# SayanoAI/Comfy-RVC

Hardware: AMD Instinct MI355X
Metric: audio-sec/wall-sec (xRT), 40k_v2 end-to-end VC (higher is better)
Workload: dtype f32; 1 GPU; Full VC 40k_v2 (HuBERT -> RMVPE -> SynthesizerTrnMs768NSFsid), 30 s 16 kHz clips, 12 per GPU per step (3 in flight), vc_single host array in -> int16 host array out (BASELINE.json configs[2]); clips_in_flight_per_gpu=3, weights=procedural (comfy-rvc_amd/synthetic.py), noise=device generator, seeded per clip, parallelism=clip-per-GPU x1 (3 lanes each), one RCCL gather of the step's int16 waveforms

## Files before the change

### comfy-rvc_amd/_lib.py

```python
import ctypes as C
import os

_HERE = os.path.dirname(os.path.abspath(__file__))
LIB_PATH = os.environ.get("RVC_HIP_LIB") or os.path.join(_HERE, "csrc", "librvc_hip.so")


class RvcHipError(RuntimeError):
    pass


def _load():
    if not os.path.isfile(LIB_PATH):
        raise RvcHipError(
            f"{LIB_PATH} is missing: build it with `python -c 'import __graft_entry__ as g; g.build()'` "
            "(or `make -C comfy-rvc_amd/csrc`).  There is no CPU fallback.")
    return C.CDLL(LIB_PATH)


lib = _load()

c_void_p, c_int, c_int64, c_float, c_char_p = C.c_void_p, C.c_int, C.c_int64, C.c_float, C.c_char_p
P = C.POINTER


# ... 38 lines not shown


SIGNATURES = {
    "rvc_last_error": (c_char_p, []),
    "rvc_version": (c_char_p, []),
    "rvc_ctx_create": (c_int, [c_int, P(c_void_p)]),
    "rvc_ctx_destroy": (c_int, [c_void_p]),
    "rvc_ctx_workspace_bytes": (c_int64, [c_void_p]),
    "rvc_ctx_set_conv_precision": (c_int, [c_void_p, c_int]),
    "rvc_hubert_create": (c_int, [c_void_p, P(c_void_p)]),
    "rvc_hubert_set_tensor": (c_int, [c_void_p, c_char_p, c_void_p, P(c_int64), c_int]),
    "rvc_hubert_finalize": (c_int, [c_void_p]),
    "rvc_hubert_destroy": (c_int, [c_void_p]),
    "rvc_hubert_num_frames": (c_int64, [c_int64]),
    "rvc_hubert_forward": (c_int, [c_void_p, c_void_p, c_void_p, c_int64, c_int, c_int, c_void_p, c_void_p, P(HubertTaps)]),
    "rvc_rmvpe_create": (c_int, [c_void_p, P(c_void_p)]),
    "rvc_rmvpe_set_tensor": (c_int, [c_void_p, c_char_p, c_void_p, P(c_int64), c_int]),
    "rvc_rmvpe_finalize": (c_int, [c_void_p]),
    "rvc_rmvpe_destroy": (c_int, [c_void_p]),
    "rvc_rmvpe_forward": (c_int, [c_void_p, c_void_p, c_void_p, c_int64, c_float, c_void_p, c_void_p, c_void_p, P(RmvpeTaps)]),
    "rvc_f0_post": (c_int, [c_void_p, c_void_p, c_int64, C.c_double, C.c_double, C.c_double, c_int, c_void_p, c_void_p]),
    "rvc_rmvpe_decode": (c_int, [c_void_p, c_void_p, c_void_p, c_int64, c_float, c_void_p]),
    "rvc_rmvpe_status": (c_int, [c_void_p, c_void_p]),
    "rvc_rmvpe_debug_fault": (c_int, [c_void_p, c_int, C.c_uint]),
    "rvc_rmvpe_repaired": (c_int, [c_void_p, c_void_p]),
    "rvc_crepe_create": (c_int, [c_void_p, c_int, P(c_void_p)]),
    "rvc_crepe_set_tensor": (c_int, [c_void_p, c_char_p, c_void_p, P(c_int64), c_int]),
    "rvc_crepe_finalize": (c_int, [c_void_p]),
    "rvc_crepe_destroy": (c_int, [c_void_p]),
    "rvc_crepe_num_frames": (c_int64, [c_int64, c_int, c_int]),
    "rvc_crepe_forward": (c_int, [c_void_p, c_void_p, c_void_p, c_int64, c_int, c_int, c_void_p, P(CrepeTaps)]),
    "rvc_crepe_viterbi": (c_int, [c_void_p, c_void_p, c_int64, c_int, c_int, c_void_p, c_void_p]),
    "rvc_mdx23_create": (c_int, [c_void_p, P(Mdx23Config), P(c_void_p)]),
    "rvc_mdx23_set_tensor": (c_int, [c_void_p, c_char_p, c_void_p, P(c_int64), c_int]),
    "rvc_mdx23_finalize": (c_int, [c_void_p]),
    "rvc_mdx23_destroy": (c_int, [c_void_p]),
    "rvc_mdx23_forward": (c_int, [c_void_p, c_void_p, c_void_p, c_int64, c_void_p]),
    "rvc_mdx23_set_streams": (c_int, [c_void_p, c_int]),
    "rvc_mdx23_demix": (c_int, [c_void_p, c_void_p, c_void_p, c_int64, c_int64, c_int64, c_float, c_void_p]),
    "rvc_synth_create": (c_int, [c_void_p, P(SynthConfig), P(c_void_p)]),
    "rvc_synth_set_tensor": (c_int, [c_void_p, c_char_p, c_void_p, P(c_int64), c_int]),
    "rvc_synth_finalize": (c_int, [c_void_p]),
    "rvc_synth_destroy": (c_int, [c_void_p]),
    "rvc_synth_upp": (c_int, [c_void_p]),
    "rvc_synth_has_f0": (c_int, [c_void_p]),
    "rvc_synth_infer": (c_int, [c_void_p, c_void_p, c_void_p, c_int, c_void_p, c_void_p, c_int, c_void_p, c_void_p, c_int64,
                                c_void_p, P(SynthTaps)]),
    "rvc_synth_infer_window": (c_int, [c_void_p, c_void_p, c_void_p, c_int, c_void_p, c_void_p, c_int, c_void_p, c_void_p, c_int64,
                                       c_void_p, P(SynthTaps), c_int64, c_int64]),
    "rvc_synth_has_posterior": (c_int, [c_void_p]),
    "rvc_synth_forward": (c_int, [c_void_p, c_void_p, c_void_p, c_int, c_void_p, c_void_p, c_void_p, c_int, c_void_p, c_void_p, c_int64, c_int64,
                                  c_void_p, P(SynthForwardTaps)]),
    "rvc_gen_tape_create": (c_int, [c_void_p, P(c_void_p)]),
    "rvc_gen_tape_release": (c_int, [c_void_p]),
    "rvc_gen_tape_bytes": (c_int64, [c_void_p]),
    "rvc_gen_tape_tensor": (c_int, [c_void_p, c_char_p, P(c_void_p), P(c_int), P(c_int64)]),
    "rvc_gen_tape_timing": (c_int, [c_void_p, c_int]),
    "rvc_gen_tape_times": (c_int, [c_void_p, P(c_float), c_int]),
    "rvc_synth_forward_tape": (c_int, [c_void_p, c_void_p, c_void_p, c_int, c_void_p, c_void_p, c_void_p, c_int, c_void_p, c_void_p, c_int64, c_int64,
                                       c_void_p, P(SynthForwardTaps), c_void_p]),
    "rvc_synth_dec_input_grad": (c_int, [c_void_p, c_void_p, c_void_p, c_void_p, c_void_p, c_void_p, c_void_p, c_void_p]),
    "rvc_synth_dec_input_grad_launch_count": (c_int, [c_void_p]),
    "rvc_synth_keep_parameters": (c_int, [c_void_p, c_int]),
    "rvc_synth_dec_param_count": (c_int, [c_void_p]),
    "rvc_synth_dec_param_info": (c_int, [c_void_p, c_int, c_char_p, c_int, P(c_int64), P(c_int)]),
    "rvc_synth_dec_param_total": (c_int64, [c_void_p]),
    "rvc_synth_dec_weight_grad": (c_int, [c_void_p, c_void_p, P(c_void_p), c_int, P(c_void_p)]),
    "rvc_synth_dec_weight_grad_launch_count": (c_int, [c_void_p]),
    "rvc_gen_tape_wgrad_times": (c_int, [c_void_p, P(c_float), c_int]),
    "rvc_conv1d_weight_grad": (c_int, [c_void_p, P(c_void_p), P(c_void_p), c_int, c_int, c_int, c_int, c_int64, c_int64, c_int, c_int, c_int, c_float, c_float,
                                       c_void_p]),
    "rvc_conv1d_weight_grad_splits": (c_int, [c_int, c_int, c_int, c_int, c_int64, c_int64, c_int, c_int, c_int]),
    "rvc_kl_loss": (c_int, [c_void_p, c_void_p, c_void_p, c_void_p, c_void_p, c_int, c_int64, c_int64, c_void_p]),
    "rvc_kl_loss_grad": (c_int, [c_void_p, c_void_p, c_void_p, c_void_p, c_int, c_int64, c_int64, c_float, c_void_p, c_void_p, c_void_p, c_void_p]),
    "rvc_l1_sum": (c_int, [c_void_p, c_void_p, c_void_p, c_int64, c_void_p]),
    "rvc_disc_create": (c_int, [c_void_p, c_int, P(c_void_p)]),
    "rvc_disc_set_tensor": (c_int, [c_void_p, c_char_p, c_void_p, P(c_int64), c_int]),
    "rvc_disc_finalize": (c_int, [c_void_p]),
    "rvc_disc_release": (c_int, [c_void_p]),
    "rvc_disc_count": (c_int, [c_void_p]),
    "rvc_disc_num_taps": (c_int, [c_void_p, c_int]),
    "rvc_disc_tap_shape": (c_int, [c_void_p, c_int, c_int, c_int64, P(c_int), P(c_int), P(c_int)]),
    "rvc_disc_forward": (c_int, [c_void_p, c_void_p, c_void_p, c_int, c_int64, P(c_void_p), P(c_void_p)]),
    "rvc_disc_launch_count": (c_int, [c_void_p, c_int, c_int64]),
    "rvc_sqerr_sums": (c_int, [c_void_p, P(c_void_p), P(c_int64), P(c_float), c_int, c_void_p]),
    "rvc_l1_sums": (c_int, [c_void_p, P(c_void_p), P(c_void_p), P(c_int64), c_int, c_void_p]),
    "rvc_disc_input_grad": (c_int, [c_void_p, c_void_p, c_int, c_int64, P(c_void_p), P(c_void_p), P(c_void_p), c_void_p]),
    "rvc_disc_input_grad_launch_count": (c_int, [c_void_p, c_int, c_int64]),
    "rvc_disc_keep_parameters": (c_int, [c_void_p, c_int]),
    "rvc_disc_param_count": (c_int, [c_void_p]),
    "rvc_disc_param_info": (c_int, [c_void_p, c_int, c_char_p, c_int, P(c_int64), P(c_int)]),
    "rvc_disc_weight_grad": (c_int, [c_void_p, c_void_p, c_void_p, c_int, c_int64, P(c_void_p), P(c_void_p), P(c_void_p)]),
    "rvc_disc_weight_grad_launch_count": (c_int, [c_void_p, c_int, c_int64]),
    "rvc_adamw_step": (c_int, [c_void_p, P(c_void_p), P(c_void_p), P(c_void_p), P(c_void_p), P(c_int64), c_int, P(AdamwHyper)]),
    "rvc_disc_adamw_step": (c_int, [c_void_p, c_void_p, c_void_p, c_void_p, c_void_p, P(AdamwHyper)]),
    "rvc_disc_adamw_step_launch_count": (c_int, [c_void_p]),
    "rvc_disc_param_total": (c_int64, [c_void_p]),
    "rvc_disc_get_parameters": (c_int, [c_void_p, c_void_p, c_void_p]),
    "rvc_disc_set_parameters": (c_int, [c_void_p, c_void_p, c_void_p]),
    "rvc_loss_cotangents": (c_int, [c_void_p, c_int, P(c_void_p), P(c_void_p), P(c_int64), P(c_float), c_int, P(c_void_p)]),
    "rvc_interpolate": (c_int, [c_void_p, c_void_p, c_void_p, c_void_p, c_int, c_int64, c_void_p]),
    "rvc_synth_dec_halo": (c_int, [c_void_p]),
    "rvc_synth_window_frames": (c_int, [c_void_p, c_int64, c_int64, c_int64, P(c_int64), P(c_int64)]),
    "rvc_synth_infer_window_halo": (c_int, [c_void_p, c_void_p, c_void_p, c_int, c_void_p, c_void_p, c_int, c_void_p, c_void_p, c_int64,
                                            c_void_p, P(SynthTaps), c_int64, c_int64, c_int]),
    "rvc_vc_segment_window": (c_int, [c_void_p, c_void_p, c_void_p, c_void_p, c_int64, c_int, c_void_p, c_void_p, c_int, c_float, c_int,
                                      c_void_p, c_void_p, c_void_p, c_int64, c_int64]),
    "rvc_vc_segment_feats_window": (c_int, [c_void_p, c_void_p, c_void_p, c_void_p, c_int64, c_int, c_void_p, c_void_p, c_int, c_float, c_int, c_void_p,
                                            c_void_p, c_void_p, c_int64, c_int64]),
    "rvc_vc_segment": (c_int, [c_void_p, c_void_p, c_void_p, c_void_p, c_int64, c_int, c_void_p, c_void_p, c_int, c_float, c_int,
                               c_void_p, c_void_p, c_void_p]),
    "rvc_vc_segment_feats": (c_int, [c_void_p, c_void_p, c_void_p, c_void_p, c_int64, c_int, c_void_p, c_void_p, c_int, c_float, c_int, c_void_p,
                                     c_void_p, c_void_p]),
    "rvc_index_create": (c_int, [c_void_p, c_void_p, c_int64, c_int, P(c_void_p)]),
    "rvc_index_create_ivf": (c_int, [c_void_p, c_void_p, c_int64, c_int, c_void_p, c_int, c_void_p, c_int, P(c_void_p)]),
    "rvc_index_nprobe": (c_int, [c_void_p]),
    "rvc_index_destroy": (c_int, [c_void_p]),
    "rvc_index_ntotal": (c_int64, [c_void_p]),
    "rvc_index_search": (c_int, [c_void_p, c_void_p, c_void_p, c_int64, c_void_p, c_void_p]),
    "rvc_index_blend": (c_int, [c_void_p, c_void_p, c_void_p, c_void_p, c_int64, c_float, c_void_p]),
    "rvc_kmeans_assign": (c_int, [c_void_p, c_void_p, c_void_p, c_int64, c_int, c_void_p, c_int, c_void_p, c_void_p]),
    "rvc_kmeans_update": (c_int, [c_void_p, c_void_p, c_void_p, c_int64, c_int, c_int, c_void_p, c_void_p]),
    "rvc_index_train": (c_int, [c_void_p, c_void_p, c_void_p, c_int64, c_int, c_void_p, c_int, c_int, c_void_p, c_void_p, c_void_p]),
    "rvc_preprocess": (c_int, [c_void_p, c_void_p, c_int, c_int64, c_void_p, c_void_p, c_void_p, c_int, c_void_p, c_void_p,
                             c_void_p, c_int, c_void_p, c_void_p]),
    "rvc_postprocess": (c_int, [c_void_p, c_void_p, c_int64, c_void_p, c_int, c_int, c_float, c_void_p]),
    "rvc_lfilter_hp": (c_int, [c_void_p, c_void_p, c_int, c_int64, c_void_p, c_void_p]),
    "rvc_frame_rms": (c_int, [c_void_p, c_void_p, c_int64, c_int, c_int, c_void_p, c_int64]),
    "rvc_slice_tags": (c_int, [c_void_p, c_int64, c_int64, C.c_double, c_int64, c_int64, c_int64, c_void_p, c_int64, P(c_int64)]),
    "rvc_cut_windows": (c_int, [c_void_p, c_void_p, c_int64, c_void_p, c_int, c_int, c_int, c_void_p, c_int, c_int, c_int, c_float, c_void_p, c_int64,
                                c_void_p, c_int64]),
    "rvc_gate_levels": (c_int, [c_void_p, c_void_p, c_int64, c_int, c_void_p, c_int64]),
    "rvc_gate_ranges": (c_int, [c_void_p, c_int64, c_int64, c_int64, c_int64, c_int64, C.c_double, c_void_p, c_int64, P(c_int64)]),
    "rvc_gate_apply": (c_int, [c_void_p, c_void_p, c_void_p, c_int64, c_void_p, c_int, c_int64]),
    "rvc_declick": (c_int, [c_void_p, c_void_p, c_int64, c_int, c_float, c_int, c_int, c_int, c_void_p, c_void_p]),
    "rvc_peak_normalize": (c_int, [c_void_p, c_void_p, c_int64, c_float, c_void_p]),
    "rvc_peak_limit": (c_int, [c_void_p, c_void_p, c_int64, c_float]),
    "rvc_merge_tracks": (c_int, [c_void_p, P(c_void_p), P(c_int64), c_int, c_int, c_void_p, c_int64]),
    "rvc_segment_energy": (c_int, [c_void_p, c_void_p, c_int64, c_int, c_void_p]),
    "rvc_spectrogram_batch": (c_int, [c_void_p, c_void_p, c_void_p, c_int64, c_void_p, c_int, c_int, c_int, c_float, c_int, c_void_p, c_int64]),
    "rvc_mel_filterbank_set": (c_int, [c_void_p, c_int, c_int, c_void_p, c_void_p, c_void_p]),
    "rvc_spec_to_mel_batch": (c_int, [c_void_p, c_void_p, c_void_p, c_int64, c_void_p, c_int, c_int, c_int, c_void_p, c_int64]),
    "rvc_spectrogram_batch_ms": (c_int, [c_void_p, c_void_p, c_void_p, c_int64, c_void_p, c_int, c_int, c_int, c_float, c_int, c_void_p, c_int64]),
    "rvc_mel_spectrogram_vjp": (c_int, [c_void_p, c_void_p, c_void_p, c_int64, c_void_p, c_int, c_int, c_int, c_float, c_int, c_int, c_void_p, c_int64,
                                        c_void_p]),
    "rvc_mel_spectrogram_vjp_launch_count": (c_int, []),
    "rvc_mel_loss_cotangents": (c_int, [c_void_p, c_int, P(c_void_p), P(c_void_p), P(c_int64), c_int, c_float, c_float, P(c_float), P(c_void_p)]),
    "rvc_multiscale_mel_loss": (c_int, [c_void_p, c_void_p, c_int, P(c_void_p), P(c_int64), P(c_int64), c_int, c_int64, P(C.c_int32), P(C.c_int32), c_int, c_int,
                                        c_void_p]),
    "rvc_hpss": (c_int, [c_void_p, c_void_p, c_int, c_int, c_int, c_void_p, c_void_p, c_int]),
    "rvc_hpss_l1": (c_int, [c_void_p, c_void_p, c_void_p, c_int, c_int, c_int, c_float, c_void_p]),
    "rvc_tsi_terms": (c_int, [c_void_p, c_void_p, c_void_p, c_int, c_int, c_int, c_float, c_void_p]),
    "rvc_op_gemm_split": (c_int, [c_void_p] * 7 + [c_int] * 4 + [c_float, c_int, c_float] + [c_int] * 5),
    "rvc_op_conv2d_split": (c_int, [c_void_p] * 7 + [c_int] * 9),
    "rvc_op_wn_in_gate_split": (c_int, [c_void_p] * 6 + [c_int] * 4),
    "rvc_op_gemm_split_qkv": (c_int, [c_void_p] * 6 + [c_int] * 4),
    "rvc_op_conv1d_s2_split": (c_int, [c_void_p] * 6 + [c_int] * 5),
    "rvc_op_conv1d_split": (c_int, [c_void_p] * 6 + [c_int] * 9),
    "rvc_op_conv1d": (c_int, [c_void_p, c_void_p, c_void_p, c_void_p, c_void_p, c_void_p] + [c_int] * 8 +
                      [c_int, c_float, c_int, c_float, c_int, c_float, c_int]),
    "rvc_op_conv_transpose1d": (c_int, [c_void_p, c_void_p, c_void_p, c_void_p, c_void_p] + [c_int] * 6 + [c_int, c_float, c_int]),
    "rvc_op_conv2d3x3": (c_int, [c_void_p, c_void_p, c_void_p, c_void_p, c_void_p, c_void_p] + [c_int] * 5),
    "rvc_op_conv_transpose2d": (c_int, [c_void_p, c_void_p, c_void_p, c_void_p, c_void_p] + [c_int] * 5),
    "rvc_op_gemm_tn": (c_int, [c_void_p, c_void_p, c_void_p, c_void_p] + [c_int] * 4),
    "rvc_conv1d_plan_create": (c_int, [c_void_p, c_void_p] + [c_int] * 7 + [P(c_void_p)]),
    "rvc_conv1d_plan_run": (c_int, [c_void_p, c_void_p, c_void_p, c_int, c_void_p, c_void_p, c_int, c_float, c_int, c_float]),
    "rvc_conv1d_plan_pair_run": (c_int, [c_void_p, c_void_p, c_void_p, c_void_p, c_int, c_void_p, c_float, c_int]),
    "rvc_conv1d_plan_resblock_run": (c_int, [P(c_void_p), c_void_p, c_void_p, c_int, c_void_p, c_float, c_int, P(c_int), c_void_p, c_void_p, c_void_p]),
    "rvc_conv1d_plan_pair_split_run": (c_int, [c_void_p, c_void_p, c_void_p, c_void_p, c_int, c_void_p, c_float, c_int]),
    "rvc_conv1d_plan_destroy": (c_int, [c_void_p]),
    "rvc_op_attention": (c_int, [c_void_p, c_void_p, c_void_p, c_void_p, c_void_p, c_void_p, c_int, c_int]),
    "rvc_op_attention_split": (c_int, [c_void_p] * 7 + [c_int, c_int]),
    "rvc_op_attention_split_rel": (c_int, [c_void_p] * 9 + [c_int, c_int, c_int]),
    "rvc_op_cbr2_small": (c_int, [c_void_p] * 7 + [c_int, c_int, c_int]),
    "rvc_op_layernorm_c_split": (c_int, [c_void_p] * 6 + [c_int, c_int]),
    "rvc_op_conv3_small": (c_int, [c_void_p] * 7 + [c_int] * 6),
    "rvc_op_gemm_split_swapped": (c_int, [c_void_p] * 4 + [c_int] * 5),
    "rvc_op_conv2d3x3_plus_1x1": (c_int, [c_void_p] * 7 + [c_int] * 6),
    "rvc_op_gemm_split_swapped_res": (c_int, [c_void_p] * 5 + [c_int] * 5),
    "rvc_op_attention_rel": (c_int, [c_void_p] * 8 + [c_int, c_int, c_void_p, c_void_p]),
    "rvc_op_layernorm_c": (c_int, [c_void_p] * 6 + [c_int, c_int]),
    "rvc_resample": (c_int, [c_void_p, c_void_p, c_int64, c_void_p, c_int, c_int, c_int, c_void_p, c_int64]),
    "rvc_set_conv_precision": (c_int, [c_int]),
    "rvc_set_pair_arithmetic": (c_int, [c_int]),
    "rvc_get_pair_arithmetic": (c_int, []),
    "rvc_conv1d_plan_pair_arithmetic": (c_int, [c_void_p, c_void_p, c_int]),
    "rvc_prof_dump_csv": (c_int, [c_char_p]),
    "rvc_prof_enable": (c_int, [c_int]),
    "rvc_prof_collect": (c_int, [P(C.c_double), P(C.c_double), P(c_int64)]),
    "rvc_prof_collect_ex": (c_int, [P(C.c_double), C.c_double, C.c_double]),
    "rvc_prof_cfg_name": (c_char_p, [c_int]),
    "rvc_op_sine_source": (c_int, [c_void_p] * 5 + [c_int, c_int, c_float, c_float, c_float] + [c_void_p] * 3),
    "rvc_op_hubert_conv0": (c_int, [c_void_p, c_void_p, c_int64, c_void_p, c_void_p, c_void_p, c_int, c_int, c_void_p, c_void_p, c_int64]),
    "rvc_op_conv_to1": (c_int, [c_void_p, c_void_p, c_int64, c_void_p, c_int, c_int, c_int, c_int, c_float, c_int, c_void_p, P(c_int)]),
    "rvc_op_noise_add": (c_int, [c_void_p, c_void_p, c_int64, c_int, c_int, c_void_p, c_int64, c_int, c_int, c_int, c_void_p, c_void_p, P(c_int)]),
    "rvc_op_transpose": (c_int, [c_void_p, c_void_p, c_void_p, c_int, c_int, c_int64, c_int64, c_int, c_int64, c_int64]),
    "rvc_op_frames": (c_int, [c_void_p, c_void_p, c_void_p] + [c_int] * 6),
    "rvc_op_mel_to_unet": (c_int, [c_void_p, c_void_p, c_void_p, c_int, c_int, c_float, c_float]),
    "rvc_op_feats_prepare": (c_int, [c_void_p] * 5 + [c_int, c_int, c_int, c_float, c_int]),
    "rvc_op_wn_gate": (c_int, [c_void_p] * 5 + [c_int, c_int]),
    "rvc_op_pool2_pad": (c_int, [c_void_p, c_void_p, c_int64, c_int, c_int, c_int, c_int, c_void_p, c_void_p, c_int64]),
    "rvc_op_interleave2_pad": (c_int, [c_void_p, c_void_p, c_int64, c_int, c_int, c_int, c_void_p, c_int, c_void_p, c_int64]),
    "rvc_op_pad2d": (c_int, [c_void_p, c_void_p, c_int64, c_int, c_int, c_int, c_void_p, c_void_p, c_int64]),
    "rvc_op_unpad2d": (c_int, [c_void_p, c_void_p, c_int64, c_int, c_int, c_int, c_void_p, c_int64]),
    "rvc_op_gru_scan": (c_int, [c_void_p] * 6 + [c_int, P(c_int)]),
}

EXPERIMENT_SIGNATURES = {
    "rvc_debug_conv_timing": (c_int, [P(C.c_uint64), c_int]),
    "rvc_debug_x3p_check": (c_int, []),
    "rvc_debug_gemm_split_bench": (c_int, [c_void_p] + [c_int] * 8 + [P(c_float), c_int, c_int]),
}

for _name, (_res, _args) in SIGNATURES.items():
    _fn = getattr(lib, _name)
    _fn.restype = _res
    _fn.argtypes = _args
has_experiments = all(hasattr(lib, _n) for _n in EXPERIMENT_SIGNATURES)
if has_experiments:
    for _name, (_res, _args) in EXPERIMENT_SIGNATURES.items():
        _fn = getattr(lib, _name)
        _fn.restype = _res
        _fn.argtypes = _args


def require_experiments():
    if not has_experiments:
        raise RuntimeError(f"{LIB_PATH} is the product library: the rvc_debug_* hooks exist in -DRVC_EXPERIMENTS builds only - "
                           "bash tools/build_variant.sh exp && RVC_HIP_LIB=comfy-rvc_amd/csrc/variants/librvc_hip_exp.so python <tool>")


def check(status):
    if status != 0:
        raise RvcHipError(lib.rvc_last_error().decode("utf-8", "replace"))


def ptr(t):
    if t is None:
        return None
    if hasattr(t, "data_ptr"):
        return c_void_p(t.data_ptr())
    return c_void_p(t.ctypes.data)


class _DeviceSpan:

    def __init__(self, address, shape):
        self.__cuda_array_interface__ = {"shape": tuple(int(v) for v in shape), "typestr": "<f4", "data": (int(address), False), "version": 2, "strides": None}


def device_view(address, shape, device):
    import torch
    with torch.cuda.device(device):
        return torch.as_tensor(_DeviceSpan(address, shape), device=device).clone()


def current_stream():
    import torch
    return c_void_p(torch.cuda.current_stream().cuda_stream)


_ctx = {}


def get_ctx(device_index=0):
    if device_index not in _ctx:
        h = c_void_p()
        check(lib.rvc_ctx_create(int(device_index), C.byref(h)))
        _ctx[device_index] = h
    return _ctx[device_index]


def set_tensors(set_fn, handle, state_dict):
    import numpy as np
    for name, v in state_dict.items():
        if hasattr(v, "detach"):
            v = v.detach().cpu()
            if not v.dtype.is_floating_point:
                continue
            v = v.float().contiguous().numpy()
        else:
            v = np.asarray(v)
            if not np.issubdtype(v.dtype, np.floating):
                continue
            v = np.ascontiguousarray(v, dtype=np.float32)
        shape = (c_int64 * max(v.ndim, 1))(*(v.shape if v.ndim else (1,)))
        check(set_fn(handle, name.encode(), c_void_p(v.ctypes.data), shape, max(v.ndim, 1)))
```

### comfy-rvc_amd/csrc/conv_x3s.hip

```cpp
#include "conv_x3_dev.h"
#include "ops.h"

namespace rvc {

struct GemmSArgs {
  const unsigned char* Wx; int CoPx;
  const unsigned char* Xs; long long xsTp;
  unsigned wx_bytes, xs_bytes;
  int Co, T, nunits;
  int ktaps, margin;
  int toff[16];
  int groups, co_g, rows_pg, cig_chunks;
  unsigned wg_bytes;
  int tdil, tpad;
  int padw; unsigned padmagic;
  const float* bias; const float* R; long long ldR;
  float* Y; long long ldY;
  unsigned char* Ys; long long ysTp;
  int act; float act_slope; int act_before_res; float out_scale;
  int ksplit; float* slabs; unsigned* tickets;
  int gx, gy;
  int xcd_remap;
  int ymargin;
  int zero_tail;
  int row_fast;
  unsigned char* Vt; long long vtTp;
  int vt_row0, vt_rows;
  const float* gate_g; int gate_h;
  int ydeint;
  int seg2_u, seg2_soff;
};

RVC_PHASE_TABLE_REGISTER;

constexpr int x3s_wgs(int AM, int AN, int RS) { return (AM * AN >= 4 && RS != 3) ? 2 : 3; }
template <int AM, int AN, int RS>
__global__ __launch_bounds__(256, x3s_wgs(AM, AN, RS)) void conv_x3s_kernel(const GemmSArgs p) {
  constexpr int WN = 2, NW = 4;
  constexpr int BM = 64 * AM, BN = 64 * AN;
  constexpr int NPA = BM / 16, NPB = BN / 16, NPW = (NPA + NPB) / NW;
  static_assert((NPA % NW) == 0 && (NPB % NW) == 0, "every wave's i-th piece is of one kind");
  constexpr int aslot = BM * 64, bslot = BN * 64, uslot = aslot + bslot;
  static_assert(RS >= 3 && (RS - 2) * NPW <= 63, "ring");
  extern __shared__ __attribute__((aligned(1024))) unsigned char smem3s[];

  const int tid0 = threadIdx.x;
  int lane = tid0 & 63;
  const int wave = __builtin_amdgcn_readfirstlane(tid0 >> 6);
  const int wm = wave / WN, wn = wave % WN;
  const int li = lane & 31, lh = lane >> 5;
  const unsigned total = gridDim.x;
  const unsigned bid = p.xcd_remap ? xcd_tile(blockIdx.x, total) : blockIdx.x;
  const int S = p.ksplit;
  const int tile = (int)(bid / (unsigned)S), ks = (int)(bid - (unsigned)tile * (unsigned)S);
  const int tile_y = p.row_fast ? tile % p.gy : tile / p.gx, tile_x = p.row_fast ? tile / p.gy : tile - tile_y * p.gx;
  const int grp = tile_y / p.rows_pg;
  const int co0 = (tile_y - grp * p.rows_pg) * BM, n0 = tile_x * BN;
  const int row0 = grp * p.co_g, CoG = p.co_g;
  const int U1 = p.nunits / S, u0 = ks * U1;
  PhaseTimer<PhaseClock::cycle> tm;
  tm.add(0, 1);

  const bool r_pre = p.R != nullptr && !(p.act_before_res && p.act != ACT_NONE);
  f32x16 acc[AM][AN];
  if (ks == 0 && (p.bias != nullptr || r_pre)) {
    const __amdgpu_buffer_rsrc_t rrs = make_rsrc(r_pre ? p.R : (const float*)p.Wx, r_pre ? (unsigned)(p.groups * p.co_g) * (unsigned)p.ldR * 4u : 0u);
#pragma unroll
    for (int am = 0; am < AM; ++am)
#pragma unroll
      for (int r = 0; r < 16; ++r) {
        const int m = co0 + (wm * AM + am) * 32 + (r & 3) + 8 * (r >> 2) + 4 * lh;
        const float bv = (p.bias && m < CoG) ? p.bias[row0 + m] : 0.f;
#pragma unroll
        for (int an = 0; an < AN; ++an) {
          const int n = n0 + (wn * AN + an) * 32 + li;
          acc[am][an][r] = buf_load(rrs, (r_pre && m < CoG && n < p.T) ? ((unsigned)(row0 + m) * (unsigned)p.ldR + (unsigned)n) * 4u : kOOB) + bv;
        }
      }
  } else {
#pragma unroll
    for (int am = 0; am < AM; ++am)
#pragma unroll
      for (int an = 0; an < AN; ++an)
#pragma unroll
        for (int r = 0; r < 16; ++r) acc[am][an][r] = 0.f;
  }

  const __amdgpu_buffer_rsrc_t ars = make_rsrc(p.Wx, p.wx_bytes), brs = make_rsrc(p.Xs, p.xs_bytes);
  int voff[NPW], dsto[NPW];
#pragma unroll
  for (int i = 0; i < NPW; ++i) {
    const int pi = wave + NW * i;
    if (i * NW < NPA) {
      constexpr int RBK = BM / 64;
      const int plane = pi / RBK, rb = pi - plane * RBK;
      voff[i] = (plane * p.CoPx + co0 + rb * 64 + lane) * 16;
      dsto[i] = plane * (BM * 16) + rb * 1024;
    } else {
      constexpr int CBK = BN / 64;
      const int pj = pi - NPA, plane = pj / CBK, cb = pj - plane * CBK;
      voff[i] = (int)((plane * p.xsTp + n0 + cb * 64 + lane) * 16);
      dsto[i] = aslot + plane * (BN * 16) + cb * 1024;
    }
  }
  const int KT = p.ktaps;
  const int wstep = p.CoPx * 64, cstep = (int)(p.xsTp * 64);
  int tap = u0 % KT;
  bool seg2 = false;
  const bool arith = KT > 16;
  auto tap_off = [&](int t) { return arith ? t * p.tdil - p.tpad : p.toff[t & 15]; };
  int soff_a = (int)((unsigned)grp * p.wg_bytes) + u0 * wstep, soff_c = (grp * p.cig_chunks + u0 / KT) * cstep, soff_b = soff_c + (p.margin + tap_off(tap)) * 16;
  if (u0 >= p.seg2_u) { seg2 = true; soff_b = p.seg2_soff + (u0 - p.seg2_u) * cstep + p.margin * 16; }
  const int seg2_at = p.seg2_u - u0;
  int slw = 0, uw = 0;
  auto issue = [&]() {
    unsigned char* base = smem3s + slw * uslot;
#pragma unroll
    for (int i = 0; i < NPW; ++i) {
      if (i * NW < NPA) buf_dma(ars, base + dsto[i], voff[i], soff_a);
      else buf_dma(brs, base + dsto[i], voff[i], soff_b);
    }
    ++uw;
    if (uw < U1) {
      soff_a += wstep;
      if (uw == seg2_at) { seg2 = true; soff_b = p.seg2_soff + p.margin * 16; }
      else if (KT > 1 && !seg2) {
        ++tap;
        if (tap == KT) { tap = 0; soff_c += cstep; }
        soff_b = soff_c + (p.margin + tap_off(tap)) * 16;
      } else {
        soff_b += cstep;
      }
    }
    slw = slw + 1 == RS ? 0 : slw + 1;
  };

  const int aoff = lh * (BM * 16) + ((wm * AM) * 32 + li) * 16;
  const int boff = aslot + lh * (BN * 16) + ((wn * AN) * 32 + li) * 16;

#pragma unroll
  for (int i = 0; i < RS - 1; ++i) issue();
  wait_vmcnt<(RS - 2) * NPW>();
#pragma unroll
  for (int am = 0; am < AM; ++am)
#pragma unroll
    for (int an = 0; an < AN; ++an) asm volatile("" : "+v"(acc[am][an]));
  lds_barrier();

  struct Ops { u32x4 ah[AM], al[AM], bh[AN], bl[AN]; };
  Ops o0, o1;
  auto read_ops = [&](Ops& o, int slot_i) {
    const unsigned char* wa = smem3s + slot_i * uslot + aoff;
    const unsigned char* xa = smem3s + slot_i * uslot + boff;
#pragma unroll
    for (int am = 0; am < AM; ++am) { o.ah[am] = *reinterpret_cast<const u32x4*>(wa + am * 512); o.al[am] = *reinterpret_cast<const u32x4*>(wa + BM * 32 + am * 512); }
#pragma unroll
    for (int an = 0; an < AN; ++an) { o.bh[an] = *reinterpret_cast<const u32x4*>(xa + an * 512); o.bl[an] = *reinterpret_cast<const u32x4*>(xa + BN * 32 + an * 512); }
  };
  auto mfmas = [&](const Ops& o) {
#pragma unroll
    for (int am = 0; am < AM; ++am)
#pragma unroll
      for (int an = 0; an < AN; ++an)
        acc[am][an] = __builtin_amdgcn_mfma_f32_32x32x16_bf16(__builtin_bit_cast(bf16x8, o.ah[am]), __builtin_bit_cast(bf16x8, o.bl[an]), acc[am][an], 0, 0, 0);
#pragma unroll
    for (int am = 0; am < AM; ++am)
#pragma unroll
      for (int an = 0; an < AN; ++an)
        acc[am][an] = __builtin_amdgcn_mfma_f32_32x32x16_bf16(__builtin_bit_cast(bf16x8, o.al[am]), __builtin_bit_cast(bf16x8, o.bh[an]), acc[am][an], 0, 0, 0);
#pragma unroll
    for (int am = 0; am < AM; ++am)
#pragma unroll
      for (int an = 0; an < AN; ++an)
        acc[am][an] = __builtin_amdgcn_mfma_f32_32x32x16_bf16(__builtin_bit_cast(bf16x8, o.ah[am]), __builtin_bit_cast(bf16x8, o.bh[an]), acc[am][an], 0, 0, 0);
  };
  int sl = 0;
  auto body = [&](const Ops& cur, Ops& nxt) {
    tm.lap(2);
    wait_vmcnt<(RS - 3) * NPW>();
    tm.lap(3);
    lds_barrier();
    tm.lap(4);
    issue();
    sl = sl + 1 == RS ? 0 : sl + 1;
    read_ops(nxt, sl);
    __builtin_amdgcn_sched_barrier(0);
    mfmas(cur);
    __builtin_amdgcn_sched_barrier(0);
  };
  read_ops(o0, 0);
  tm.lap(1);
  int u = 0;
  for (; u + 1 < U1; u += 2) { body(o0, o1); body(o1, o0); }
  if (u < U1) body(o0, o1);
  tm.lap(2);
  asm volatile("s_waitcnt vmcnt(0)" ::: "memory");
  tm.mark();

  if (S > 1) {
    typedef float f32x4_t __attribute__((ext_vector_type(4)));
    constexpr int QN = AM * AN * 4;
    const unsigned slab_bytes = 256u * QN * 16u;
    const __amdgpu_buffer_rsrc_t srs = make_rsrc(p.slabs, (unsigned)(total) * slab_bytes);
    const unsigned lane_off = ((unsigned)wave * QN * 64u + (unsigned)lane) * 16u;
    {
      const unsigned mine = ((unsigned)tile * (unsigned)S + (unsigned)ks) * slab_bytes + lane_off;
#pragma unroll
      for (int am = 0; am < AM; ++am)
#pragma unroll
        for (int an = 0; an < AN; ++an)
#pragma unroll
          for (int q = 0; q < 4; ++q) {
            const u32x4 v = {__float_as_uint(acc[am][an][4 * q]), __float_as_uint(acc[am][an][4 * q + 1]), __float_as_uint(acc[am][an][4 * q + 2]),
                             __float_as_uint(acc[am][an][4 * q + 3])};
            __builtin_amdgcn_raw_buffer_store_b128(v, srs, (int)(mine + (unsigned)(((am * AN + an) * 4 + q) * 64) * 16u), 0, 16);
          }
    }
    asm volatile("s_waitcnt vmcnt(0)" ::: "memory");
    __syncthreads();
    unsigned* flag = reinterpret_cast<unsigned*>(smem3s);
    if (tid0 == 0) {
      const unsigned t = __hip_atomic_fetch_add(p.tickets + tile, 1u, __ATOMIC_RELAXED, __HIP_MEMORY_SCOPE_AGENT);
      if (t == (unsigned)S - 1u) __hip_atomic_store(p.tickets + tile, 0u, __ATOMIC_RELAXED, __HIP_MEMORY_SCOPE_AGENT);
      *flag = t;
    }
    __syncthreads();
    tm.lap(5); tm.flush();
    if (*flag != (unsigned)S - 1u) return;
#pragma unroll
    for (int am = 0; am < AM; ++am)
#pragma unroll
      for (int an = 0; an < AN; ++an)
#pragma unroll
        for (int q = 0; q < 4; ++q) {
          f32x4_t own = {acc[am][an][4 * q], acc[am][an][4 * q + 1], acc[am][an][4 * q + 2], acc[am][an][4 * q + 3]};
          f32x4_t sum = {0.f, 0.f, 0.f, 0.f};
          for (int z = 0; z < S; ++z) {
            f32x4_t v = own;
            if (z != ks) {
              const unsigned off = ((unsigned)tile * (unsigned)S + (unsigned)z) * slab_bytes + lane_off + (unsigned)(((am * AN + an) * 4 + q) * 64) * 16u;
              const u32x4 w = __builtin_amdgcn_raw_buffer_load_b128(srs, (int)off, 0, 16);
              v = f32x4_t{__uint_as_float(w[0]), __uint_as_float(w[1]), __uint_as_float(w[2]), __uint_as_float(w[3])};
            }
            sum = z == 0 ? v : sum + v;
          }
#pragma unroll
          for (int j = 0; j < 4; ++j) acc[am][an][4 * q + j] = sum[j];
        }
  }

  const float oscale = p.out_scale;
  if (p.act == ACT_GELU) {
#pragma unroll
    for (int am = 0; am < AM; ++am)
#pragma unroll
      for (int an = 0; an < AN; ++an)
#pragma unroll
        for (int r = 0; r < 16; ++r) acc[am][an][r] = gelu_bf(acc[am][an][r]);
  } else if (p.act != ACT_NONE) {
    const float slope = p.act == ACT_RELU ? 0.f : p.act_slope;
#pragma unroll
    for (int am = 0; am < AM; ++am)
#pragma unroll
      for (int an = 0; an < AN; ++an)
#pragma unroll
        for (int r = 0; r < 16; ++r) { const float v = acc[am][an][r]; acc[am][an][r] = fmaxf(v, v * slope); }
  }
  if (p.R != nullptr && !r_pre) {
    const __amdgpu_buffer_rsrc_t rrs2 = make_rsrc(p.R, (unsigned)(p.groups * p.co_g) * (unsigned)p.ldR * 4u);
#pragma unroll
    for (int am = 0; am < AM; ++am)
#pragma unroll
      for (int an = 0; an < AN; ++an) {
        const int n = n0 + (wn * AN + an) * 32 + li;
        float rv[16];
#pragma unroll
        for (int r = 0; r < 16; ++r) {
          const int m = co0 + (wm * AM + am) * 32 + (r & 3) + 8 * (r >> 2) + 4 * lh;
          rv[r] = buf_load(rrs2, (m < CoG && n < p.T) ? ((unsigned)(row0 + m) * (unsigned)p.ldR + (unsigned)n) * 4u : kOOB);
        }
#pragma unroll
        for (int r = 0; r < 16; ++r) acc[am][an][r] += rv[r];
      }
  }
  if (oscale != 1.f) {
#pragma unroll
    for (int am = 0; am < AM; ++am)
#pragma unroll
      for (int an = 0; an < AN; ++an)
#pragma unroll
        for (int r = 0; r < 16; ++r) acc[am][an][r] *= oscale;
  }
  if (p.padw > 0) {
#pragma unroll
    for (int an = 0; an < AN; ++an) {
      const unsigned n = (unsigned)(n0 + (wn * AN + an) * 32 + li);
      const unsigned q = __umulhi(n, p.padmagic), w = n - q * (unsigned)p.padw;
      if (w == 0u || w == (unsigned)p.padw - 1u) {
#pragma unroll
        for (int am = 0; am < AM; ++am)
#pragma unroll
          for (int r = 0; r < 16; ++r) acc[am][an][r] = 0.f;
      }
    }
  }
  const bool vt_tile = co0 >= p.vt_row0;
  if (vt_tile) {
    typedef float f32x4v __attribute__((ext_vector_type(4)));
    unsigned char* tl = smem3s + 1024 + wave * 4096;
    const int Tc16 = (p.T + 15) & ~15;
#pragma unroll
    for (int am = 0; am < AM; ++am)
#pragma unroll
      for (int an = 0; an < AN; ++an) {
        const int nb = n0 + (wn * AN + an) * 32;
#pragma unroll
        for (int r = 0; r < 16; ++r) {
          const int jj = (r & 3) + 8 * (r >> 2) + 4 * lh;
          *reinterpret_cast<float*>(tl + (jj * 32 + li) * 4) = (nb + li < p.T) ? acc[am][an][r] : 0.f;
        }
        asm volatile("s_waitcnt lgkmcnt(0)" ::: "memory");
#pragma unroll
        for (int it = 0; it < 2; ++it) {
          const int item = lane + 64 * it, jj = item >> 2, tg = item & 3;
          const f32x4v va = *reinterpret_cast<const f32x4v*>(tl + (jj * 32 + tg * 8) * 4), vb = *reinterpret_cast<const f32x4v*>(tl + (jj * 32 + tg * 8 + 4) * 4);
          u32x4 hi, lo;
          unsigned h_, l_;
          split2(va[0], va[1], h_, l_); hi[0] = h_; lo[0] = l_;
          split2(va[2], va[3], h_, l_); hi[1] = h_; lo[1] = l_;
          split2(vb[0], vb[1], h_, l_); hi[2] = h_; lo[2] = l_;
          split2(vb[2], vb[3], h_, l_); hi[3] = h_; lo[3] = l_;
          const int t0 = nb + tg * 8, j = co0 + (wm * AM + am) * 32 + jj - p.vt_row0;
          if (t0 < Tc16 && j < p.vt_rows) {
            unsigned char* row = p.Vt + ((((long long)(t0 >> 4)) * 4 + ((t0 >> 3) & 1)) * p.vtTp + kSplitMargin + j) * 16;
            *reinterpret_cast<u32x4*>(row) = hi;
            *reinterpret_cast<u32x4*>(row + p.vtTp * 32) = lo;
          }
        }
        asm volatile("s_waitcnt lgkmcnt(0)" ::: "memory");
      }
  }
  if (p.Y && !vt_tile) {
    const __amdgpu_buffer_rsrc_t yrs = make_rsrc(p.Y, (unsigned)(p.groups * p.co_g) * (unsigned)p.ldY * 4u);
#pragma unroll
    for (int am = 0; am < AM; ++am)
#pragma unroll
      for (int r = 0; r < 16; ++r) {
        const int m = co0 + (wm * AM + am) * 32 + (r & 3) + 8 * (r >> 2) + 4 * lh;
#pragma unroll
        for (int an = 0; an < AN; ++an) {
          const int n = n0 + (wn * AN + an) * 32 + li;
          __builtin_amdgcn_raw_buffer_store_b32(__float_as_uint(acc[am][an][r]), yrs, (int)((m < CoG && n < p.T) ? ((unsigned)(row0 + m) * (unsigned)p.ldY + (unsigned)n) * 4u : kOOB), 0, 0);
        }
      }
  }
  if (p.Ys && p.gate_h > 0) {
    const int H = p.gate_h;
#pragma unroll
    for (int am = 0; am < AM; ++am) {
      const int blk = (co0 + (wm * AM + am) * 32) >> 5;
      float gt[8], gsg[8];
#pragma unroll
      for (int r = 0; r < 8; ++r) {
        const int c = 16 * blk + (r & 3) + 8 * (r >> 2) + 4 * lh;
        gt[r] = (p.gate_g && c < H) ? p.gate_g[c] : 0.f; gsg[r] = (p.gate_g && c < H) ? p.gate_g[H + c] : 0.f;
      }
#pragma unroll
      for (int an = 0; an < AN; ++an) {
        const int n = n0 + (wn * AN + an) * 32 + li;
        float v[8];
#pragma unroll
        for (int r = 0; r < 8; ++r) {
          constexpr float kL2E = 1.44269504088896340736f;
          const float ta = acc[am][an][r] + gt[r], sa = acc[am][an][r + 8] + gsg[r];
          const float th = 1.f - 2.f * __builtin_amdgcn_rcpf(__builtin_amdgcn_exp2f(2.f * kL2E * ta) + 1.f);
          v[r] = th * __builtin_amdgcn_rcpf(1.f + __builtin_amdgcn_exp2f(-kL2E * sa));
        }
        unsigned hA[2], lA[2], hB[2], lB[2];
#pragma unroll
        for (int e2 = 0; e2 < 2; ++e2) {
          split2(v[2 * e2], v[2 * e2 + 1], hA[e2], lA[e2]);
          split2(v[4 + 2 * e2], v[5 + 2 * e2], hB[e2], lB[e2]);
        }
        u32x4 hi, lo;
#pragma unroll
        for (int e2 = 0; e2 < 2; ++e2) {
          typedef unsigned u32x2_t __attribute__((ext_vector_type(2)));
          const u32x2_t sh = __builtin_amdgcn_permlane32_swap(hA[e2], hB[e2], false, false);
          const u32x2_t sl2 = __builtin_amdgcn_permlane32_swap(lA[e2], lB[e2], false, false);
          hi[e2] = sh.x; hi[2 + e2] = sh.y; lo[e2] = sl2.x; lo[2 + e2] = sl2.y;
        }
        if (n < p.T && 16 * blk < H) {
          unsigned char* row = p.Ys + (((long long)blk * 4 + lh) * p.ysTp + (long long)n + p.ymargin) * 16;
          *reinterpret_cast<u32x4*>(row) = hi;
          *reinterpret_cast<u32x4*>(row + p.ysTp * 32) = lo;
        }
      }
    }
  } else if (p.Ys && !vt_tile) {
    if (p.zero_tail) {
#pragma unroll
      for (int am = 0; am < AM; ++am)
#pragma unroll
        for (int r = 0; r < 16; ++r) {
          const int m = co0 + (wm * AM + am) * 32 + (r & 3) + 8 * (r >> 2) + 4 * lh;
          if (m >= CoG) {
#pragma unroll
            for (int an = 0; an < AN; ++an) acc[am][an][r] = 0.f;
          }
        }
    }
#pragma unroll
    for (int am = 0; am < AM; ++am)
#pragma unroll
      for (int an = 0; an < AN; ++an) {
        const int n = n0 + (wn * AN + an) * 32 + li;
        const int mb = co0 + (wm * AM + am) * 32;
        const long long pos = p.ydeint > 0 ? (long long)p.ymargin + (n >> 1) + (long long)(n & 1) * p.ydeint : (long long)n + p.ymargin;
#pragma unroll
        for (int g2 = 0; g2 < 2; ++g2) {
          unsigned hA[2], lA[2], hB[2], lB[2];
#pragma unroll
          for (int e2 = 0; e2 < 2; ++e2) {
            split2(acc[am][an][8 * g2 + 2 * e2], acc[am][an][8 * g2 + 2 * e2 + 1], hA[e2], lA[e2]);
            split2(acc[am][an][8 * g2 + 4 + 2 * e2], acc[am][an][8 * g2 + 5 + 2 * e2], hB[e2], lB[e2]);
          }
          u32x4 hi, lo;
#pragma unroll
          for (int e2 = 0; e2 < 2; ++e2) {
            typedef unsigned u32x2_t __attribute__((ext_vector_type(2)));
            const u32x2_t sh = __builtin_amdgcn_permlane32_swap(hA[e2], hB[e2], false, false);
            const u32x2_t sl2 = __builtin_amdgcn_permlane32_swap(lA[e2], lB[e2], false, false);
            hi[e2] = sh.x; hi[2 + e2] = sh.y; lo[e2] = sl2.x; lo[2 + e2] = sl2.y;
          }
          if (n < p.T && mb + 16 * g2 < CoG) {
            const long long chunk = ((row0 + mb) >> 4) + g2;
            unsigned char* row = p.Ys + ((chunk * 4 + lh) * p.ysTp + pos) * 16;
            *reinterpret_cast<u32x4*>(row) = hi;
            *reinterpret_cast<u32x4*>(row + p.ysTp * 32) = lo;
          }
        }
      }
  }
  tm.lap(5); tm.flush();
}

__global__ __launch_bounds__(256) void split_image_kernel(const float* __restrict__ X, long long ldX, int C, int T, unsigned char* __restrict__ img, long long tp) {
  const int t = blockIdx.x * 256 + threadIdx.x;
  const int hp = blockIdx.y;
  if (t >= T) return;
  const float* x = X + (long long)(hp * 8) * ldX + t;
  u32x4 hi, lo;
#pragma unroll
  for (int j = 0; j < 4; ++j) {
    const float a = (hp * 8 + 2 * j) < C ? x[(long long)(2 * j) * ldX] : 0.f, b = (hp * 8 + 2 * j + 1) < C ? x[(long long)(2 * j + 1) * ldX] : 0.f;
    unsigned h_, l_;
    split2(a, b, h_, l_);
    hi[j] = h_; lo[j] = l_;
  }
  const int chunk = hp >> 1, half = hp & 1;
  unsigned char* row = img + (((long long)chunk * 4 + half) * tp + kSplitMargin + t) * 16;
  *reinterpret_cast<u32x4*>(row) = hi;
  *reinterpret_cast<u32x4*>(row + tp * 32) = lo;
}
__global__ __launch_bounds__(256) void unsplit_image_kernel(const unsigned char* __restrict__ img, long long tp, int C, int T, float* __restrict__ Y, long long ldY) {
  const int t = blockIdx.x * 256 + threadIdx.x;
  const int hp = blockIdx.y;
  if (t >= T) return;
  const int chunk = hp >> 1, half = hp & 1;
  const unsigned char* row = img + (((long long)chunk * 4 + half) * tp + kSplitMargin + t) * 16;
  const u32x4 hi = *reinterpret_cast<const u32x4*>(row), lo = *reinterpret_cast<const u32x4*>(row + tp * 32);
#pragma unroll
  for (int j = 0; j < 4; ++j) {
    const int c = hp * 8 + 2 * j;
    if (c < C) Y[(long long)c * ldY + t] = __uint_as_float(hi[j] << 16) + __uint_as_float(lo[j] << 16);
    if (c + 1 < C) Y[(long long)(c + 1) * ldY + t] = __uint_as_float(hi[j] & 0xffff0000u) + __uint_as_float(lo[j] & 0xffff0000u);
  }
}
void split_image_from_f32(hipStream_t s, const float* X, long long ldX, int C, int T, unsigned char* img, long long tp) {
  hipLaunchKernelGGL(split_image_kernel, dim3((T + 255) / 256, (C + 15) / 16 * 2), dim3(256), 0, s, X, ldX, C, T, img, tp);
}
__global__ __launch_bounds__(256) void split_image_tm_kernel(const float* __restrict__ x, int C, int T, int M, unsigned char* __restrict__ img, long long tp) {
  typedef float f32x4_t __attribute__((ext_vector_type(4)));
  const int t = blockIdx.x * 256 + threadIdx.x;
  const int hp = blockIdx.y;
  if (t >= T) return;
  const int f0 = hp * 8, c = f0 / M, m0 = f0 - c * M;
  u32x4 hi, lo;
  if (c < C) {
    const float* src = x + ((long long)c * T + t) * M + m0;
    const f32x4_t a = *reinterpret_cast<const f32x4_t*>(src), b = *reinterpret_cast<const f32x4_t*>(src + 4);
    unsigned h_, l_;
    split2(a[0], a[1], h_, l_); hi[0] = h_; lo[0] = l_;
    split2(a[2], a[3], h_, l_); hi[1] = h_; lo[1] = l_;
    split2(b[0], b[1], h_, l_); hi[2] = h_; lo[2] = l_;
    split2(b[2], b[3], h_, l_); hi[3] = h_; lo[3] = l_;
  } else {
    hi = u32x4{0u, 0u, 0u, 0u}; lo = hi;
  }
  unsigned char* row = img + (((long long)(hp >> 1) * 4 + (hp & 1)) * tp + kSplitMargin + t) * 16;
  *reinterpret_cast<u32x4*>(row) = hi;
  *reinterpret_cast<u32x4*>(row + tp * 32) = lo;
}
void split_image_from_tm(hipStream_t s, const float* x, int C, int T, int M, unsigned char* img, long long tp) {
  RVC_REQUIRE((M & 7) == 0 && (reinterpret_cast<uintptr_t>(x) & 15) == 0, "split_image_from_tm: rows of a multiple of 8 values, 16-byte aligned");
  hipLaunchKernelGGL(split_image_tm_kernel, dim3((T + 255) / 256, (C * M + 15) / 16 * 2), dim3(256), 0, s, x, C, T, M, img, tp);
}
__global__ __launch_bounds__(256) void split_image_deint_kernel(const float* __restrict__ X, long long ldX, int C, int T, unsigned char* __restrict__ img, long long tp, int H) {
  const int t = blockIdx.x * 256 + threadIdx.x;
  const int hp = blockIdx.y;
  if (t >= T) return;
  const float* x = X + (long long)(hp * 8) * ldX + t;
  u32x4 hi, lo;
#pragma unroll
  for (int j = 0; j < 4; ++j) {
    const float a = (hp * 8 + 2 * j) < C ? x[(long long)(2 * j) * ldX] : 0.f, b = (hp * 8 + 2 * j + 1) < C ? x[(long long)(2 * j + 1) * ldX] : 0.f;
    unsigned h_, l_;
    split2(a, b, h_, l_);
    hi[j] = h_; lo[j] = l_;
  }
  unsigned char* row = img + (((long long)(hp >> 1) * 4 + (hp & 1)) * tp + kSplitMargin + (t >> 1) + (long long)(t & 1) * H) * 16;
  *reinterpret_cast<u32x4*>(row) = hi;
  *reinterpret_cast<u32x4*>(row + tp * 32) = lo;
}
__global__ __launch_bounds__(256) void unsplit_image_deint_kernel(const unsigned char* __restrict__ img, long long tp, int H, int C, int T, float* __restrict__ Y, long long ldY) {
  const int t = blockIdx.x * 256 + threadIdx.x;
  const int hp = blockIdx.y;
  if (t >= T) return;
  const unsigned char* row = img + (((long long)(hp >> 1) * 4 + (hp & 1)) * tp + kSplitMargin + (t >> 1) + (long long)(t & 1) * H) * 16;
  const u32x4 hi = *reinterpret_cast<const u32x4*>(row), lo = *reinterpret_cast<const u32x4*>(row + tp * 32);
#pragma unroll
  for (int j = 0; j < 4; ++j) {
    const int c = hp * 8 + 2 * j;
    if (c < C) Y[(long long)c * ldY + t] = __uint_as_float(hi[j] << 16) + __uint_as_float(lo[j] << 16);
    if (c + 1 < C) Y[(long long)(c + 1) * ldY + t] = __uint_as_float(hi[j] & 0xffff0000u) + __uint_as_float(lo[j] & 0xffff0000u);
  }
}
void split_image_deint_from_f32(hipStream_t s, const float* X, long long ldX, int C, int T, unsigned char* img, long long tp, int H) {
  hipLaunchKernelGGL(split_image_deint_kernel, dim3((T + 255) / 256, (C + 15) / 16 * 2), dim3(256), 0, s, X, ldX, C, T, img, tp, H);
}
void split_image_deint_to_f32(hipStream_t s, const unsigned char* img, long long tp, int H, int C, int T, float* Y, long long ldY) {
  hipLaunchKernelGGL(unsplit_image_deint_kernel, dim3((T + 255) / 256, (C + 15) / 16 * 2), dim3(256), 0, s, img, tp, H, C, T, Y, ldY);
}
void split_image_to_f32(hipStream_t s, const unsigned char* img, long long tp, int C, int T, float* Y, long long ldY) {
  hipLaunchKernelGGL(unsplit_image_kernel, dim3((T + 255) / 256, (C + 15) / 16 * 2), dim3(256), 0, s, img, tp, C, T, Y, ldY);
}

template <int AM, int AN, int RS>
static void launch_x3s(const GemmSArgs& a, unsigned blocks, hipStream_t s) {
  auto kern = conv_x3s_kernel<AM, AN, RS>;
  constexpr size_t lds = (size_t)RS * (64 * AM + 64 * AN) * 64;
  RVC_ALLOW_BIG_LDS(kern);
  conv_launch(kern, dim3(blocks), dim3(256), lds, s, a);
}
static void x3s_dispatch(const GemmSArgs& a, int AM, int AN, unsigned blocks, hipStream_t s) {
  const bool rs3 = AM == 2 && AN == 2 && blocks >= 768u && a.nunits / a.ksplit >= 64;
  if (AM == 2 && AN == 2) { if (rs3) launch_x3s<2, 2, 3>(a, blocks, s); else launch_x3s<2, 2, 4>(a, blocks, s); }
  else if (AM == 2 && AN == 1) launch_x3s<2, 1, 4>(a, blocks, s);
  else if (AM == 1 && AN == 2) launch_x3s<1, 2, 4>(a, blocks, s);
  else launch_x3s<1, 1, 4>(a, blocks, s);
}

static thread_local int t_force_s = 0, t_force_am = 0, t_force_an = 0;
void conv_x3s_force(int ksplit, int am, int an) { t_force_s = ksplit; t_force_am = am; t_force_an = an; }
static void x3s_plan(int M, long long Nplan, int units, int& AM, int& AN, int& S, int groups = 1) {
  static const int target = exp_int("RVC_X3S_BLK", 440);
  auto tiles = [&](int am, int an) { return (long long)groups * ((M + 64 * am - 1) / (64 * am)) * ((Nplan + 64 * an - 1) / (64 * an)); };
  AM = 2; AN = 2;
  const bool deep = units >= 128 && groups == 1 && tiles(2, 2) >= 256;
  if (!deep && tiles(AM, AN) < target) AN = 1;
  if (!deep && tiles(AM, AN) < target) AM = 1;
  if (groups > 1) AM = 1;
  if ((t_force_am == 1 || t_force_am == 2) && groups == 1) AM = t_force_am;
  if (t_force_an == 1 || t_force_an == 2) AN = t_force_an;
  S = 1;
  const long long nt = tiles(AM, AN);
  static const int min_units = exp_int("RVC_X3S_MINUNITS", 32);
  for (int c : {2, 3, 4, 6, 8, 12, 16}) {
    if (nt * S >= target) break;
    if (units % c == 0 && units / c >= min_units) S = c;
  }
  if (t_force_s > 0) S = (units % t_force_s == 0 && units / t_force_s >= 4) ? t_force_s : 1;
}

bool conv_x3s_eligible(const ConvLayer& L) {
  if (L.Wx_ == nullptr || (L.Ci & 15) != 0 || L.Ci * L.ktaps < 32 || L.tconv_u != 0 || L.up2 != 0) return false;
  if (L.mode == 2) return L.ktaps <= 16;
  if (L.mode != 1 || L.stride != 1 || L.pad > kSplitMargin || (L.k - 1) * L.dil - L.pad > kSplitMargin) return false;
  if (L.groups > 1) return (L.Co & 15) == 0 && (L.CoPx & 63) == 0 && L.CoPx <= 64;
  return L.k <= 16 && L.pad == (L.k - 1) / 2 * L.dil && (L.k & 1) == 1;
}

SplitGeom split_geom_s2(int k, long long Tin) {
  SplitGeom g; g.ktaps = k; g.s2_h = split_s2_h(Tin); g.margin = kSplitMargin; g.padw = 0;
  RVC_REQUIRE(k >= 1 && k <= 16, "split_geom_s2: at most 16 taps");
  for (int t = 0; t < k; ++t) g.toff[t] = (t & 1) * g.s2_h + (t >> 1);
  return g;
}
bool conv_x3s_s2_eligible(const ConvLayer& L) {
  return L.Wx_ != nullptr && L.mode == 1 && L.stride == 2 && L.pad == 0 && L.dil == 1 && L.groups == 1 && L.tconv_u == 0 && L.up2 == 0 &&
         (L.Ci & 15) == 0 && (L.Co & 15) == 0 && L.k >= 2 && L.k <= 16 && L.seg2_chunks == 0;
}

SplitGeom split_geom_2d(int Wd, int KH, int KW, int PH, int PWL) {
  SplitGeom g; g.padw = Wd + 2; g.ktaps = KH * KW;
  RVC_REQUIRE(g.ktaps <= 16 && PWL <= 1 && KW - 1 - PWL <= 1, "split_geom_2d: at most one pad column on each side");
  for (int kh = 0; kh < KH; ++kh) for (int kw = 0; kw < KW; ++kw) g.toff[kh * KW + kw] = (kh - PH) * g.padw + (kw - PWL);
  int maxoff = 0;
  for (int t = 0; t < g.ktaps; ++t) maxoff = std::max(maxoff, std::abs(g.toff[t]));
  g.margin = kSplitMargin;
  while (g.margin < maxoff) g.margin += 64;
  return g;
}

void conv_x3s_run(const ConvLayer& L, hipStream_t s, const unsigned char* Xs, long long xsTp, int T, float* Y, long long ldY, const ConvEpilogue& e,
                  const SplitGeom* geom) {
  const bool s2 = geom != nullptr && geom->s2_h > 0;
  RVC_REQUIRE(s2 ? conv_x3s_s2_eligible(L) : conv_x3s_eligible(L), "conv_x3s_run: layer without a bf16x3 weight image or not a stride-1 'same' (stride-2 'valid' with a de-interleaved image) geometry");
  SplitGeom g1;
  if (!geom) {
    RVC_REQUIRE(L.mode == 1, "conv_x3s_run: a 2-D layer needs its padded-image geometry");
    g1.ktaps = L.k; g1.margin = kSplitMargin; g1.padw = 0;
    for (int t = 0; t < L.k && t < 16; ++t) g1.toff[t] = t * L.dil - L.pad;
    geom = &g1;
  }
  RVC_REQUIRE(geom->ktaps == L.ktaps || (L.mode == 1 && geom->ktaps == L.k), "conv_x3s_run: geometry and layer disagree about the taps");
  if (s2) {
    RVC_REQUIRE(Xs != nullptr && xsTp >= geom->margin + 2LL * geom->s2_h + 704 && (long long)T + 1 <= geom->s2_h, "conv_x3s_run: de-interleaved input image missing or too short");
  } else {
  int maxoff = L.mode == 1 ? std::max(L.pad, (L.k - 1) * L.dil - L.pad) : 0;
  for (int t = 0; t < geom->ktaps && t < 16; ++t) maxoff = std::max(maxoff, std::abs(geom->toff[t]));
  RVC_REQUIRE(geom->margin >= maxoff && geom->margin >= kSplitMargin, "conv_x3s_run: image margin smaller than the largest tap offset");
  RVC_REQUIRE(Xs != nullptr && xsTp >= geom->margin + T + 704, "conv_x3s_run: split-resident input image missing or too short (margin + T + 704 rows per plane)");
  }
  RVC_REQUIRE(Y != nullptr || e.ys_out != nullptr, "conv_x3s_run: no output");
  RVC_REQUIRE(e.pre_act == ACT_NONE && !e.accumulate && !e.tout_limit && !e.xs_in, "conv_x3s_run: unsupported epilogue option");
  RVC_REQUIRE(e.plan_tin == 0 || (!s2 && L.mode == 1 && e.plan_tin >= T), "conv_x3s_run: a column window is a window of a longer 1-D 'same' convolution");
  RVC_REQUIRE(e.act == ACT_NONE || e.act == ACT_LRELU || e.act == ACT_RELU || e.act == ACT_GELU, "conv_x3s_run: activation must be identity / (leaky) ReLU / GELU");
  RVC_REQUIRE(!e.ys_out || ((e.ys_deint_h > 0 ? (e.ys_tp >= geom->margin + 2LL * e.ys_deint_h + 704 && (T + 1) / 2 + 1 <= e.ys_deint_h) : e.ys_tp >= geom->margin + T + 704) && (L.Co & 15) == 0),
              "conv_x3s_run: split output image too short or Co not a multiple of 16");
  RVC_REQUIRE((double)L.groups * L.Co * (double)(Y ? ldY : 1) * 4.0 < 2147483648.0 && (double)L.groups * L.Co * (double)e.ldR * 4.0 < 2147483648.0, "tensor extent exceeds 32-bit buffer addressing");
  const int G = L.mode == 1 ? L.groups : 1;
  RVC_REQUIRE(L.seg2_chunks == 0 || (G == 1 && geom->seg2_off > 0), "conv_x3s_run: a layer with an appended product needs its second image");
  const double xs_bytes = std::max((double)G * (L.Ci / 16) * 4.0 * (double)xsTp * 16.0, L.seg2_chunks ? (double)geom->seg2_off + (double)L.seg2_chunks * 4.0 * (double)xsTp * 16.0 : 0.0);
  const double wx_bytes = (double)G * (L.Ci / 16) * geom->ktaps * 4.0 * (double)L.CoPx * 16.0 + (double)L.seg2_chunks * 4.0 * (double)L.CoPx * 16.0;
  RVC_REQUIRE(G == 1 || (!e.ys_out || (L.Co & 15) == 0), "grouped layer: rows per group must be a multiple of 16 for the image output");
  RVC_REQUIRE(xs_bytes < 2147483648.0 && wx_bytes < 2147483648.0, "operand image exceeds 32-bit buffer addressing");
  GemmSArgs a{};
  a.Wx = reinterpret_cast<const unsigned char*>(L.Wx_); a.CoPx = L.CoPx; a.Xs = Xs; a.xsTp = xsTp;
  a.wx_bytes = (unsigned)wx_bytes; a.xs_bytes = (unsigned)xs_bytes;
  a.Co = L.Co; a.T = T; a.nunits = L.Ci / 16 * geom->ktaps + L.seg2_chunks;
  a.seg2_u = L.seg2_chunks ? L.Ci / 16 * geom->ktaps : 0x7fffffff; a.seg2_soff = (int)geom->seg2_off;
  a.ktaps = geom->ktaps; a.margin = geom->margin; a.ymargin = geom->margin; a.padw = geom->padw; a.ydeint = e.ys_out ? e.ys_deint_h : 0;
  if (e.gate_h > 0) {
    RVC_REQUIRE(G == 1 && L.mode == 1 && L.Co == 2 * e.gate_h && (e.gate_h & 15) == 0 && e.ys_out && Y == nullptr && !e.R && e.act == ACT_NONE && e.out_scale == 1.f && !e.vt_out && !e.ys_deint_h,
                "conv_x3s_run: the gate epilogue wants a 2 H-row layer packed by wn_gate_row_order, an image output and nothing else");
    a.gate_h = e.gate_h; a.gate_g = e.gate_g;
  }
  a.vt_row0 = 0x7fffffff;
  if (e.vt_out) {
    RVC_REQUIRE(G == 1 && L.mode == 1 && e.vt_row0 > 0 && (e.vt_row0 & 127) == 0 && e.vt_row0 < L.Co && e.vt_tp >= kSplitMargin + (L.Co - e.vt_row0) && Y == nullptr && !e.R && !s2,
                "conv_x3s_run: the transposed rows are the tail of an image-only k = 1 projection, from a multiple of 128 rows on");
    a.Vt = e.vt_out; a.vtTp = e.vt_tp; a.vt_row0 = e.vt_row0; a.vt_rows = L.Co - e.vt_row0;
  }
  a.padmagic = geom->padw > 0 ? (unsigned)((0x100000000ULL + (unsigned)geom->padw - 1) / (unsigned)geom->padw) : 0u;
  for (int t = 0; t < 16; ++t) a.toff[t] = t < geom->ktaps ? geom->toff[t] : 0;
  a.tdil = L.mode == 1 ? L.dil : 1; a.tpad = L.mode == 1 ? L.pad : 0;
  if (s2) { a.tdil = 1; a.tpad = 0; }
  a.groups = G; a.co_g = L.Co; a.cig_chunks = L.Ci / 16; a.wg_bytes = (unsigned)((double)(L.Ci / 16) * geom->ktaps * 4.0 * (double)L.CoPx * 16.0);
  a.bias = e.bias_override ? e.bias_override : L.bd_; a.R = e.R; a.ldR = e.ldR; a.Y = Y; a.ldY = ldY; a.Ys = e.ys_out; a.ysTp = e.ys_tp;
  a.act = e.act; a.act_slope = e.act_slope; a.act_before_res = e.act_before_res; a.out_scale = e.out_scale;
  int AM, AN, S;
  x3s_plan(L.Co, e.plan_tin > 0 ? e.plan_tin : T, a.nunits, AM, AN, S, G);
  const int BM = 64 * AM, BN = 64 * AN;
  RVC_REQUIRE(L.CoPx % BM == 0, "weight image rows are padded to the tile");
  a.rows_pg = (L.Co + BM - 1) / BM;
  a.gx = (T + BN - 1) / BN; a.gy = a.rows_pg * G; a.ksplit = S;
  a.xcd_remap = x3_xcd_remap();
  const unsigned blocks = (unsigned)((long long)a.gx * a.gy * S);
  if (S > 1) {
    const size_t slab_bytes = (size_t)blocks * BM * BN * 4;
    const size_t tick_bytes = ((size_t)a.gx * a.gy * 4 + 255) & ~(size_t)255;
    static const size_t kTickCap = 64 * 1024;
    RVC_REQUIRE(tick_bytes <= kTickCap, "too many tiles for the ticket array");
    bool fresh = false;
    a.tickets = (unsigned*)stream_scratch_zeroed(s, 7, kTickCap, &fresh);
    a.slabs = (float*)stream_scratch(s, 6, slab_bytes);
  }
  ProfTicket tk = conv_prof_begin(s);
  x3s_dispatch(a, AM, AN, blocks, s);
  if (tk.on) {
    ConvArgsX pa{};
    pa.Ci = L.Ci; pa.Co = L.Co; pa.ktaps = geom->ktaps; pa.kreal = geom->ktaps; pa.dil = L.mode == 1 ? L.dil : 1; pa.stride = s2 ? 2 : 1; pa.Tin = T; pa.Tout = T;
    pa.Wd = geom->padw > 0 ? geom->padw - 2 : 0; pa.ksplit = S;
    pa.R = e.R; pa.X = nullptr;
    const double bytes = 4.0 * ((double)L.Ci * T + (double)L.Co * T * ((Y ? 1.0 : 0.0) + (e.ys_out ? 1.0 : 0.0) + (e.R ? 1.0 : 0.0)) + (double)L.Co * L.Ci * geom->ktaps);
    const int id = AM == 2 ? (AN == 2 ? 3 : 5) : (AN == 2 ? 5 : 6);
    conv_prof_end(tk, s, 2.0 * (double)G * L.Co * T * (L.Ci * geom->ktaps + 16 * L.seg2_chunks), 14 + id, bytes * (G > 1 ? (double)G : 1.0), &pa, (long long)blocks, 4 << 4);
  }
}

void conv_x3s_run_swapped(const ConvLayer& L, int row0, int rows, hipStream_t s, const unsigned char* Xs, long long xsTp, int T, unsigned char* Ys, long long ysTp,
                          float* Yrm, long long ldYrm, const float* Rrm, long long ldRrm) {
  RVC_REQUIRE(L.Wx_ != nullptr && L.mode == 1 && L.k == 1 && L.groups == 1 && (L.Ci & 15) == 0, "conv_x3s_run_swapped: a k = 1 projection with a bf16x3 weight image");
  RVC_REQUIRE(row0 >= 0 && rows > 0 && row0 + rows <= L.Co && (row0 & 15) == 0, "conv_x3s_run_swapped: row range");
  RVC_REQUIRE(Xs != nullptr && xsTp >= kSplitMargin + T + 704 && (Ys != nullptr || Yrm != nullptr) && (!Ys || ysTp >= kSplitMargin + rows), "conv_x3s_run_swapped: images missing or too short");
  RVC_REQUIRE(!Yrm || (ldYrm >= rows && (double)T * (double)ldYrm * 4.0 < 2147483648.0), "conv_x3s_run_swapped: row-major output pitch");
  RVC_REQUIRE(!Rrm || (Yrm && ldRrm >= rows && (double)T * (double)ldRrm * 4.0 < 2147483648.0), "conv_x3s_run_swapped: the residual goes with the row-major output");
  const double xs_bytes = (double)(L.Ci / 16) * 4.0 * (double)xsTp * 16.0, wx_bytes = (double)(L.Ci / 16) * 4.0 * (double)L.CoPx * 16.0;
  RVC_REQUIRE(xs_bytes < 2147483648.0 && wx_bytes < 2147483648.0, "operand image exceeds 32-bit buffer addressing");
  GemmSArgs a{};
  a.Wx = Xs + (size_t)kSplitMargin * 16; a.CoPx = (int)xsTp; a.wx_bytes = (unsigned)xs_bytes - (unsigned)kSplitMargin * 16u;
  a.Xs = reinterpret_cast<const unsigned char*>(L.Wx_) + (size_t)row0 * 16; a.xsTp = L.CoPx; a.xs_bytes = (unsigned)wx_bytes - (unsigned)row0 * 16u;
  a.Co = T; a.T = rows; a.nunits = L.Ci / 16; a.ktaps = 1; a.margin = 0; a.ymargin = kSplitMargin; a.zero_tail = 1; a.seg2_u = 0x7fffffff; a.vt_row0 = 0x7fffffff;
  a.groups = 1; a.co_g = T; a.cig_chunks = L.Ci / 16; a.tdil = 1;
  a.Ys = Ys; a.ysTp = ysTp; a.act = ACT_NONE; a.out_scale = 1.f;
  a.Y = Yrm; a.ldY = ldYrm;
  a.R = Rrm; a.ldR = ldRrm;
  int AM, AN, S;
  x3s_plan(T, rows, a.nunits, AM, AN, S);
  S = 1;
  const int BM = 64 * AM, BN = 64 * AN;
  RVC_REQUIRE((long long)((T + BM - 1) / BM) * BM <= xsTp - kSplitMargin && (long long)row0 + (long long)((rows + BN - 1) / BN) * BN <= L.CoPx, "conv_x3s_run_swapped: a tile would read past an operand image");
  a.rows_pg = (T + BM - 1) / BM; a.gx = (rows + BN - 1) / BN; a.gy = a.rows_pg; a.ksplit = 1;
  a.xcd_remap = x3_xcd_remap();
  const unsigned blocks = (unsigned)((long long)a.gx * a.gy);
  ProfTicket tk = conv_prof_begin(s);
  x3s_dispatch(a, AM, AN, blocks, s);
  if (tk.on) {
    ConvArgsX pa{};
    pa.Ci = L.Ci; pa.Co = rows; pa.ktaps = 1; pa.kreal = 1; pa.dil = 1; pa.stride = 1; pa.Tin = T; pa.Tout = T; pa.ksplit = 1;
    const double bytes = 4.0 * ((double)L.Ci * T + (double)rows * T * (Rrm ? 2.0 : 1.0) + (double)rows * L.Ci);
    const int id = AM == 2 ? (AN == 2 ? 3 : 5) : (AN == 2 ? 5 : 6);
    conv_prof_end(tk, s, 2.0 * (double)rows * T * L.Ci, 14 + id, bytes, &pa, (long long)blocks, 4 << 4);
  }
}

}
```

### comfy-rvc_amd/csrc/rvc_api.hip

```cpp
#include "models.h"
#include "conv_kernels.h"

namespace rvc {
static thread_local std::string g_err;
void set_error(const std::string& msg) { g_err = msg; }
}

using namespace rvc;

struct rvc_ctx { Ctx c; };
static std::mutex g_ctx_mu;
static std::map<int, int> g_ctx_count;
struct rvc_hubert { Hubert* m; rvc_ctx* ctx; };
struct rvc_rmvpe { Rmvpe* m; rvc_ctx* ctx; };
struct rvc_synth { Synth* m; rvc_ctx* ctx; };
struct rvc_conv1d_plan { OwnedConvLayer L; };

#define RVC_TRY try {
#define RVC_CATCH                                                            \
  return 0;                                                                  \
  }                                                                          \
  catch (const std::exception& e) { rvc::set_error(e.what()); return 1; }    \
  catch (...) { rvc::set_error("unknown error"); return 2; }

struct X3sForceScope {
  X3sForceScope(int ksplit, int am, int an) { conv_x3s_force(ksplit, am, an); }
  ~X3sForceScope() { conv_x3s_force(0, 0, 0); }
  X3sForceScope(const X3sForceScope&) = delete; X3sForceScope& operator=(const X3sForceScope&) = delete;
};
struct AttentionKzScope {
  explicit AttentionKzScope(int kz) { attention_split_force_kz(kz); }
  ~AttentionKzScope() { attention_split_force_kz(0); }
  AttentionKzScope(const AttentionKzScope&) = delete; AttentionKzScope& operator=(const AttentionKzScope&) = delete;
};
typedef DevBuf<unsigned char> DevBytes;
static DevBytes image_from_f32(hipStream_t s, const float* x, int C, int T, int fill) {
  DevBytes img;
  img.alloc(split_image_bytes(C, T));
  RVC_HIP_CHECK(hipMemsetAsync(img.p, fill, split_image_bytes(C, T), s));
  split_image_from_f32(s, x, T, C, T, img.p, split_image_tp(T));
  return img;
}

static void attention_operand_images(hipStream_t s, const float* q, const float* k, const float* v, int C, int T, DevBytes& qk, DevBuf<float>& vtf, DevBytes& vt) {
  const long long tp = split_image_tp(T), vtp = attention_vt_tp(C);
  qk.alloc(split_image_bytes(2 * C, T));
  RVC_HIP_CHECK(hipMemsetAsync(qk.p, 0xff, split_image_bytes(2 * C, T), s));
  split_image_from_f32(s, q, T, C, T, qk.p, tp);
  split_image_from_f32(s, k, T, C, T, qk.p + split_image_bytes(C, T), tp);
  vtf.alloc((size_t)T * C);
  transpose(s, v, vtf.p, C, T, T, C, 1, 0, 0);
  vt.alloc(attention_vt_bytes(C, T));
  RVC_HIP_CHECK(hipMemsetAsync(vt.p, 0xff, attention_vt_bytes(C, T), s));
  split_image_from_f32(s, vtf.p, C, T, C, vt.p, vtp);
  attention_vt_clear_tail(s, vt.p, C, T);
}

static void check_launch() {
  hipError_t e = hipGetLastError();
  if (e != hipSuccess) throw Error(std::string("kernel launch failed: ") + hipGetErrorString(e));
}

extern "C" {

const char* rvc_last_error(void) { return g_err.c_str(); }
const char* rvc_version(void) { return "rvc_hip 0.1.0 (gfx950, fp32 MFMA)"; }

int rvc_ctx_create(int device_id, rvc_ctx** out) {
  RVC_TRY
  int n = 0;
  RVC_HIP_CHECK(hipGetDeviceCount(&n));
  RVC_REQUIRE(n > 0 && device_id >= 0 && device_id < n, "no such HIP device (this library has no CPU path)");
  RVC_HIP_CHECK(hipSetDevice(device_id));
  hipDeviceProp_t prop;
  RVC_HIP_CHECK(hipGetDeviceProperties(&prop, device_id));
  RVC_REQUIRE(std::string(prop.gcnArchName).find("gfx950") != std::string::npos,
              std::string("kernels are built for gfx950 only, found ") + prop.gcnArchName);
  rvc_ctx* c = new rvc_ctx();
  c->c.device = device_id;
  { std::lock_guard<std::mutex> lk(g_ctx_mu); ++g_ctx_count[device_id]; }
  *out = c;
  RVC_CATCH
}
int rvc_ctx_destroy(rvc_ctx* ctx) {
  if (!ctx) return 0;
  bool last;
  { std::lock_guard<std::mutex> lk(g_ctx_mu); last = --g_ctx_count[ctx->c.device] <= 0; }
  if (last) { (void)hipSetDevice(ctx->c.device); stream_scratch_release(ctx->c.device); }
  spec_state_free(&ctx->c);
  delete ctx;
  return 0;
}
int rvc_ctx_set_conv_precision(rvc_ctx* ctx, int mode) {
  RVC_TRY
  RVC_REQUIRE(ctx && mode >= -1 && mode <= 2, "precision mode must be -1 (thread default), 0, 1 or 2");
  ctx->c.precision = mode;
  RVC_CATCH
}
int64_t rvc_ctx_workspace_bytes(rvc_ctx* ctx) { return ctx ? (int64_t)ctx->c.workspace_bytes : 0; }

int rvc_hubert_create(rvc_ctx* ctx, rvc_hubert** out) {
  RVC_TRY
  RVC_REQUIRE(ctx && out, "null argument");
  rvc_hubert* h = new rvc_hubert(); h->ctx = ctx; h->m = hubert_create(&ctx->c); *out = h;
  RVC_CATCH
}
int rvc_hubert_set_tensor(rvc_hubert* h, const char* name, const float* d, const int64_t* shape, int ndim) {
  RVC_TRY
  RVC_REQUIRE(h && name && d && ndim <= 8, "bad argument");
  long long sh[8]; for (int i = 0; i < ndim; ++i) sh[i] = shape[i];
  hubert_set_tensor(h->m, name, d, sh, ndim);
  RVC_CATCH
}
int rvc_hubert_finalize(rvc_hubert* h) { RVC_TRY RVC_REQUIRE(h, "null argument"); RVC_HIP_CHECK(hipSetDevice(h->ctx->c.device)); hubert_finalize(h->m); RVC_CATCH }
int rvc_hubert_destroy(rvc_hubert* h) { if (h) { hubert_destroy(h->m); delete h; } return 0; }
int64_t rvc_hubert_num_frames(int64_t L) { return hubert_num_frames(L); }
int rvc_hubert_forward(rvc_hubert* h, void* stream, const float* audio, int64_t L, int version, int n_layers, float* out_rm, float* out_cm,
                       const rvc_hubert_taps* taps) {
  RVC_TRY
  RVC_REQUIRE(h && audio, "null argument");
  hubert_forward(h->m, (hipStream_t)stream, audio, L, version, n_layers, out_rm, out_cm, taps);
  check_launch();
  h->ctx->c.workspace_bytes = hubert_workspace(h->m);
  RVC_CATCH
}

int rvc_rmvpe_create(rvc_ctx* ctx, rvc_rmvpe** out) {
  RVC_TRY
  RVC_REQUIRE(ctx && out, "null argument");
  rvc_rmvpe* r = new rvc_rmvpe(); r->ctx = ctx; r->m = rmvpe_create(&ctx->c); *out = r;
  RVC_CATCH
}
int rvc_rmvpe_set_tensor(rvc_rmvpe* r, const char* name, const float* d, const int64_t* shape, int ndim) {
  RVC_TRY
  RVC_REQUIRE(r && name && d && ndim <= 8, "bad argument");
  long long sh[8]; for (int i = 0; i < ndim; ++i) sh[i] = shape[i];
  rmvpe_set_tensor(r->m, name, d, sh, ndim);
  RVC_CATCH
}
int rvc_rmvpe_finalize(rvc_rmvpe* r) { RVC_TRY RVC_REQUIRE(r, "null argument"); RVC_HIP_CHECK(hipSetDevice(r->ctx->c.device)); rmvpe_finalize(r->m); RVC_CATCH }
int rvc_rmvpe_destroy(rvc_rmvpe* r) { if (r) { rmvpe_destroy(r->m); delete r; } return 0; }
int rvc_rmvpe_forward(rvc_rmvpe* r, void* stream, const float* audio, int64_t L, float thred, float* mel, float* sal, double* f0,
                      const rvc_rmvpe_taps* taps) {
  RVC_TRY
  RVC_REQUIRE(r && audio, "null argument");
  rmvpe_forward(r->m, (hipStream_t)stream, audio, L, thred, mel, sal, f0, taps);
  check_launch();
  RVC_CATCH
}
int rvc_rmvpe_status(rvc_rmvpe* r, void* stream) {
  RVC_TRY
  RVC_REQUIRE(r, "null argument");
  RVC_REQUIRE(rmvpe_status(r->m, (hipStream_t)stream) != 1,
              "RMVPE: the GRU scan's workgroups timed out waiting for each other (they need to be co-resident) and the repair pass did not run; the f0 of the last forward is invalid (NaN)");
  RVC_CATCH
}
int rvc_rmvpe_repaired(rvc_rmvpe* r, void* stream) { return (r && r->m && rmvpe_status(r->m, (hipStream_t)stream) == 2) ? 1 : 0; }
int rvc_rmvpe_debug_fault(rvc_rmvpe* r, int fault, unsigned spin_limit) { RVC_TRY RVC_REQUIRE(r, "null argument"); rmvpe_debug_fault(r->m, fault, spin_limit); RVC_CATCH }
int rvc_rmvpe_decode(rvc_rmvpe* r, void* stream, const float* sal, int64_t n, float thred, double* f0) {
  RVC_TRY
  RVC_REQUIRE(r && sal && f0 && n > 0, "bad argument");
  rmvpe_decode_rm(r->m, (hipStream_t)stream, sal, n, thred, f0);
  check_launch();
  RVC_CATCH
}
int rvc_f0_post(void* stream, const double* f0, int64_t n, double factor, double mel_min, double mel_max, int bins, int64_t* pitch, float* pitchf) {
  RVC_TRY
  RVC_REQUIRE(f0 && pitch && pitchf && n > 0 && bins > 2 && mel_max > mel_min, "bad argument");
  f0_post((hipStream_t)stream, f0, n, factor, mel_min, mel_max, bins, reinterpret_cast<long long*>(pitch), pitchf);
  check_launch();
  RVC_CATCH
}

struct rvc_crepe { Crepe* m; rvc_ctx* ctx; };
int rvc_crepe_create(rvc_ctx* ctx, int tiny, rvc_crepe** out) {
  RVC_TRY
  RVC_REQUIRE(ctx && out, "null argument");
  std::unique_ptr<rvc_crepe> c(new rvc_crepe()); c->ctx = ctx; c->m = crepe_create(&ctx->c, tiny);
  *out = c.release();
  RVC_CATCH
// ... 592 lines not shown
                    int64_t* ranges, int64_t cap, int64_t* n_ranges) {
  RVC_TRY
  RVC_REQUIRE(level && ranges && n_ranges && n > 0 && win > 0 && cap >= 0, "bad argument");
  RVC_REQUIRE(n_windows == (n + win - 1) / win, "level must hold ceil(n / win) windows");
  RVC_REQUIRE(fade >= 2 && min_size >= 2 * fade, "fade >= 2 samples and min_size >= 2 fade");
  *n_ranges = gate_ranges(level, n_windows, n, win, min_size, fade, threshold_db, (long long*)ranges, cap);
  RVC_CATCH
}
int rvc_gate_apply(void* stream, const float* x, float* y, int64_t n, const int64_t* ranges, int n_ranges, int64_t fade) {
  RVC_TRY
  RVC_REQUIRE(x && y && n > 0 && n_ranges >= 0 && (ranges || n_ranges == 0) && fade >= 2, "bad argument");
  gate_apply((hipStream_t)stream, x, y, n, (const long long*)ranges, n_ranges, fade);
  check_launch();
  RVC_CATCH
}
int rvc_declick(void* stream, const float* x, int64_t n, int size, float multiplier, int method, int kernel_size, int detect, float* y, uint8_t* mask) {
  RVC_TRY
  if (!detect) size = 1;
  RVC_REQUIRE(x && y && mask && n > 0 && size > 0 && (method == 0 || method == 1) && multiplier >= 0.f, "bad argument");
  RVC_REQUIRE(kernel_size >= 1 && (kernel_size & 1) && kernel_size <= kMaxClickKernel, "kernel_size must be odd and at most 31");
  RVC_REQUIRE(n >= size && n >= kernel_size, "the signal must be at least as long as the RMS window and the median window");
  RVC_REQUIRE(x != y, "declick reads the unmodified input: y must not be x");
  declick((hipStream_t)stream, x, n, size, multiplier, method, kernel_size, detect != 0, y, mask);
  check_launch();
  RVC_CATCH
}
int rvc_peak_normalize(void* stream, const float* x, int64_t n, float gain, float* y) {
  RVC_TRY
  RVC_REQUIRE(x && y && n > 0 && gain > 0.f, "bad argument");
  peak_normalize((hipStream_t)stream, x, n, gain, y);
  check_launch();
  RVC_CATCH
}
int rvc_peak_limit(void* stream, float* x, int64_t n, float max_volume) {
  RVC_TRY
  RVC_REQUIRE(x && n > 0 && max_volume > 0.f, "bad argument");
  peak_limit((hipStream_t)stream, x, n, max_volume);
  check_launch();
  RVC_CATCH
}
int rvc_merge_tracks(void* stream, const float* const* tracks, const int64_t* lens, int k, int mode, float* out, int64_t n_out) {
  RVC_TRY
  RVC_REQUIRE(tracks && lens && out && k >= 2 && k <= 4 && mode >= 0 && mode <= 3 && n_out > 0, "bad argument");
  long long l[4];
  for (int j = 0; j < k; ++j) {
    RVC_REQUIRE(lens[j] >= 0 && lens[j] <= n_out && (tracks[j] || lens[j] == 0), "every track must fit the output");
    l[j] = lens[j];
  }
  merge_tracks((hipStream_t)stream, tracks, l, k, mode, out, n_out);
  check_launch();
  RVC_CATCH
}
int rvc_segment_energy(void* stream, const int16_t* x, int64_t n, int k, int64_t* out) {
  RVC_TRY
  RVC_REQUIRE(x && out && k >= 1 && n >= k, "bad argument");
  segment_energy((hipStream_t)stream, x, n, k, (long long*)out);
  check_launch();
  RVC_CATCH
}

int rvc_spectrogram_batch(rvc_ctx* ctx, void* stream, const float* audio, int64_t n_audio, const int64_t* clips, int n_clips, int n_fft, int hop, float eps,
                          int clamp, float* out, int64_t pitch) {
  RVC_TRY
  RVC_REQUIRE(ctx && audio && out && (clips || n_clips == 0), "null argument");
  spectrogram_batch(&ctx->c, (hipStream_t)stream, audio, n_audio, (const long long*)clips, n_clips, n_fft, hop, eps, clamp, out, pitch);
  check_launch();
  RVC_CATCH
}
int rvc_mel_filterbank_set(rvc_ctx* ctx, int n_fft, int n_mels, const int32_t* first, const int32_t* count, const float* weights) {
  RVC_TRY
  RVC_REQUIRE(ctx, "null argument");
  RVC_HIP_CHECK(hipSetDevice(ctx->c.device));
  mel_filterbank_set(&ctx->c, n_fft, n_mels, (const int*)first, (const int*)count, weights);
  RVC_CATCH
}
int rvc_spec_to_mel_batch(rvc_ctx* ctx, void* stream, const float* spec, int64_t spec_pitch, const int64_t* clips, int n_clips, int n_fft, int n_mels,
                          float* mel, int64_t mel_pitch) {
  RVC_TRY
  RVC_REQUIRE(ctx && spec && mel && (clips || n_clips == 0), "null argument");
  spec_to_mel_batch(&ctx->c, (hipStream_t)stream, spec, spec_pitch, (const long long*)clips, n_clips, n_fft, n_mels, mel, mel_pitch);
  check_launch();
  RVC_CATCH
}
int rvc_spectrogram_batch_ms(rvc_ctx* ctx, void* stream, const float* audio, int64_t n_audio, const int64_t* clips, int n_clips, int n_fft, int hop, float eps,
                             int clamp, float* out, int64_t pitch) {
  RVC_TRY
  RVC_REQUIRE(ctx && audio && out && (clips || n_clips == 0), "null argument");
  spectrogram_batch_ms(&ctx->c, (hipStream_t)stream, audio, n_audio, (const long long*)clips, n_clips, n_fft, hop, eps, clamp, out, pitch);
  check_launch();
  RVC_CATCH
}
int rvc_mel_spectrogram_vjp(rvc_ctx* ctx, void* stream, const float* audio, int64_t n_audio, const int64_t* clips, int n_clips, int n_fft, int hop, float eps,
                            int clamp, int n_mels, const float* cot_mel, int64_t pitch, float* d_audio) {
  RVC_TRY
  RVC_REQUIRE(ctx && audio && cot_mel && d_audio && (clips || n_clips == 0), "null argument");
  mel_spectrogram_vjp(&ctx->c, (hipStream_t)stream, audio, n_audio, (const long long*)clips, n_clips, n_fft, hop, eps, clamp, n_mels, cot_mel, pitch, d_audio);
  check_launch();
  RVC_CATCH
}
int rvc_mel_spectrogram_vjp_launch_count(void) { return kMelVjpLaunches; }
int rvc_mel_loss_cotangents(void* stream, int K, const float* const* a, const float* const* b, const int64_t* n, int loss, float log_weight, float mag_weight,
                            const float* scale, float* const* out) {
  RVC_TRY
  mel_loss_cotangents((hipStream_t)stream, K, a, b, (const long long*)n, loss, log_weight, mag_weight, scale, out);
  check_launch();
  RVC_CATCH
}
int rvc_multiscale_mel_loss(rvc_ctx* ctx, void* stream, int K, const float* const* spec, const int64_t* pitch, const int64_t* row_stride, int B, int64_t nf,
                            const int32_t* n_fft, const int32_t* n_mels, int loss, int want_mag, double* out) {
  RVC_TRY
  RVC_REQUIRE(ctx && spec && pitch && row_stride && n_fft && n_mels && out, "null argument");
  multiscale_mel_loss(&ctx->c, (hipStream_t)stream, K, spec, (const long long*)pitch, (const long long*)row_stride, B, nf, (const int*)n_fft, (const int*)n_mels,
                      loss, want_mag, out);
  check_launch();
  RVC_CATCH
}

int rvc_hpss(void* stream, const float* x, int B, int F, int T, float* h, float* p, int medians) {
  RVC_TRY
  hpss_parts((hipStream_t)stream, x, B, F, T, h, p, medians);
  check_launch();
  RVC_CATCH
}
int rvc_hpss_l1(void* stream, const float* org, const float* gen, int B, int F, int T, float eps, double* sums) {
  RVC_TRY
  hpss_l1((hipStream_t)stream, org, gen, B, F, T, eps, sums);
  check_launch();
  RVC_CATCH
}
int rvc_tsi_terms(void* stream, const float* org, const float* gen, int B, int F, int T, float eps, double* out) {
  RVC_TRY
  tsi_terms((hipStream_t)stream, org, gen, B, F, T, eps, out);
  check_launch();
  RVC_CATCH
}

int rvc_op_conv1d(void* stream, const float* x, const float* w, const float* bias, const float* res, float* y, int Ci, int Co, int Tin, int k,
                  int stride, int pad, int dil, int groups, int pre_act, float pre_slope, int act, float act_slope, int act_before_res,
                  float out_scale, int accumulate) {
  RVC_TRY
  OwnedConvLayer L;
  conv1d_layer_init(L, w, bias, Co, Ci, k, stride, pad, dil, groups);
  ConvEpilogue e; e.pre_act = pre_act; e.pre_slope = pre_slope; e.act = act; e.act_slope = act_slope; e.act_before_res = act_before_res;
  e.out_scale = out_scale; e.accumulate = accumulate;
  const int Tout = conv1d_out_len(L, Tin);
  e.R = res; e.ldR = Tout;
  conv1d_run(L, (hipStream_t)stream, x, Tin, Tin, y, Tout, e);
  check_launch();
  RVC_HIP_CHECK(hipStreamSynchronize((hipStream_t)stream));
  RVC_CATCH
}
int rvc_op_gemm_split(void* stream, const float* x, const float* w, const float* bias, const float* res, float* y, float* ysplit_f32, int Ci, int Co,
                      int T, int act, float act_slope, int act_before_res, float out_scale, int ksplit, int am, int an, int k, int dil) {
  RVC_TRY
  RVC_REQUIRE(x && w && (y || ysplit_f32) && Ci > 0 && Co > 0 && T > 0 && k >= 1 && (k & 1) == 1 && dil >= 1, "bad argument");
  hipStream_t s = (hipStream_t)stream;
  OwnedConvLayer L;
  { ConvBuildScope scope(2); conv1d_layer_init(L, w, bias, Co, Ci, k, 1, (k - 1) / 2 * dil, dil, 1); }
  RVC_REQUIRE(conv_x3s_eligible(L), "layer not eligible for the split-resident GEMM (Ci % 16 == 0, Ci k >= 64, Co >= 32, pad <= 64)");
  const long long tp = split_image_tp(T);
  DevBytes xs = image_from_f32(s, x, Ci, T, 0), ys;
  ConvEpilogue e; e.act = act; e.act_slope = act_slope; e.act_before_res = act_before_res; e.out_scale = out_scale; e.R = res; e.ldR = T;
  if (ysplit_f32) { ys.alloc(split_image_bytes(Co, T)); e.ys_out = ys.p; e.ys_tp = tp; }
  { X3sForceScope force(ksplit, am, an); conv_x3s_run(L, s, xs.p, tp, T, y, T, e); }
  if (ysplit_f32) split_image_to_f32(s, ys.p, tp, Co, T, ysplit_f32, T);
  check_launch();
  RVC_HIP_CHECK(hipStreamSynchronize(s));
  RVC_CATCH
}
int rvc_op_gemm_split_swapped(void* stream, const float* x, const float* w, float* yt, int Ci, int Co, int T, int row0, int rows) {
  RVC_TRY
  RVC_REQUIRE(x && w && yt && Ci > 0 && Co > 0 && T > 0 && rows > 0, "bad argument");
  hipStream_t s = (hipStream_t)stream;
  OwnedConvLayer L;
  { ConvBuildScope scope(2); conv1d_layer_init(L, w, nullptr, Co, Ci, 1, 1, 0, 1, 1); }
  const long long tp = split_image_tp(T), vtp = attention_vt_tp(rows);
  const size_t vbytes = attention_vt_bytes(rows, T);
  DevBytes xs = image_from_f32(s, x, Ci, T, 0xff), ys;
  ys.alloc(vbytes);
  RVC_HIP_CHECK(hipMemsetAsync(ys.p, 0xff, vbytes, s));
  conv_x3s_run_swapped(L, row0, rows, s, xs.p, tp, T, ys.p, vtp);
  attention_vt_clear_tail(s, ys.p, rows, T);
  split_image_to_f32(s, ys.p, vtp, (T + 63) / 64 * 64, rows, yt, rows);
  check_launch();
  RVC_HIP_CHECK(hipStreamSynchronize(s));
  RVC_CATCH
}
int rvc_op_wn_in_gate_split(void* stream, const float* x, const float* w, const float* bias, const float* g_dev, float* y, int Ci, int H, int T, int k) {
  RVC_TRY
  RVC_REQUIRE(x && w && y && Ci > 0 && H > 0 && (H & 15) == 0 && T > 0 && k >= 1 && (k & 1) == 1, "bad argument");
  hipStream_t s = (hipStream_t)stream;
  std::vector<float> wp((size_t)2 * H * Ci * k), bp((size_t)2 * H, 0.f);
  for (int r = 0; r < 2 * H; ++r) {
    const int src = wn_gate_row_order(r, H);
    std::copy(w + (size_t)src * Ci * k, w + (size_t)(src + 1) * Ci * k, wp.begin() + (size_t)r * Ci * k);
    if (bias) bp[r] = bias[src];
  }
  OwnedConvLayer L;
  { ConvBuildScope scope(2); conv1d_layer_init(L, wp.data(), bp.data(), 2 * H, Ci, k, 1, (k - 1) / 2, 1, 1); }
  RVC_REQUIRE(conv_x3s_eligible(L), "layer not eligible for the split-resident kernel");
  const long long tp = split_image_tp(T);
  DevBytes xs = image_from_f32(s, x, Ci, T, 0), ys;
  ys.alloc(split_image_bytes(H, T));
  ConvEpilogue e; e.ys_out = ys.p; e.ys_tp = tp; e.gate_h = H; e.gate_g = g_dev;
  conv_x3s_run(L, s, xs.p, tp, T, nullptr, T, e);
  split_image_to_f32(s, ys.p, tp, H, T, y, T);
  check_launch();
  RVC_HIP_CHECK(hipStreamSynchronize(s));
  RVC_CATCH
}
int rvc_op_gemm_split_qkv(void* stream, const float* x, const float* w, const float* bias, float* y_img_f32, float* yt, int Ci, int Co, int T, int vt_row0) {
  RVC_TRY
  RVC_REQUIRE(x && w && y_img_f32 && yt && Ci > 0 && Co > 0 && T > 0 && vt_row0 > 0 && vt_row0 < Co, "bad argument");
  hipStream_t s = (hipStream_t)stream;
  OwnedConvLayer L;
  { ConvBuildScope scope(2); conv1d_layer_init(L, w, bias, Co, Ci, 1, 1, 0, 1, 1); }
  const int rows = Co - vt_row0;
  RVC_REQUIRE(conv_x3s_eligible(L), "layer not eligible for the split-resident kernel");
  const long long tp = split_image_tp(T), vtp = attention_vt_tp(rows);
  const size_t vbytes = attention_vt_bytes(rows, T);
  DevBytes xs = image_from_f32(s, x, Ci, T, 0xff), ys, vt;
  ys.alloc(split_image_bytes(vt_row0, T));
  vt.alloc(vbytes);
  RVC_HIP_CHECK(hipMemsetAsync(vt.p, 0xff, vbytes, s));
  ConvEpilogue e; e.ys_out = ys.p; e.ys_tp = tp; e.vt_out = vt.p; e.vt_tp = vtp; e.vt_row0 = vt_row0;
  conv_x3s_run(L, s, xs.p, tp, T, nullptr, T, e);
  attention_vt_clear_tail(s, vt.p, rows, T);
  split_image_to_f32(s, ys.p, tp, vt_row0, T, y_img_f32, T);
  split_image_to_f32(s, vt.p, vtp, (T + 63) / 64 * 64, rows, yt, rows);
  check_launch();
  RVC_HIP_CHECK(hipStreamSynchronize(s));
  RVC_CATCH
}
int rvc_op_conv2d3x3_plus_1x1(void* stream, const float* x1, const float* w1, const float* x2, const float* w2, float* y, float* y_img_f32, int Ci1, int Ci2, int Co, int H, int W,
                              int ksplit) {
  RVC_TRY
  RVC_REQUIRE(x1 && w1 && x2 && w2 && y && Ci1 > 0 && Ci2 > 0 && Co > 0 && H > 0 && W > 0, "bad argument");
  hipStream_t s = (hipStream_t)stream;
  OwnedConvLayer L1, L2;
  { ConvBuildScope scope(2); conv2d3x3_layer_init(L1, w1, nullptr, Co, Ci1); conv1d_layer_init(L2, w2, nullptr, Co, Ci2, 1, 1, 0, 1, 1); }
  RVC_REQUIRE(conv_x3s_eligible(L1) && conv_x3s_eligible(L2), "layers not eligible for the split-resident GEMM (channels % 16, Co >= 32)");
  conv_layer_append_x3(L1, L2);
  SplitGeom g = split_geom_2d(W);
  const long long TP = (long long)H * (W + 2), tp = ((long long)g.margin + TP + std::max(704, g.margin) + 63) & ~63LL;
  const size_t b1 = (size_t)(Ci1 / 16) * 4 * (size_t)tp * 16, b2 = (size_t)(Ci2 / 16) * 4 * (size_t)tp * 16, bo = (size_t)((Co + 15) / 16) * 4 * (size_t)tp * 16;
  DevBytes img, yimg; DevBuf<float> yp;
  img.alloc(b1 + b2); RVC_HIP_CHECK(hipMemsetAsync(img.p, 0, b1 + b2, s));
  yp.alloc((size_t)Co * TP);
  if (y_img_f32) { yimg.alloc(bo); RVC_HIP_CHECK(hipMemsetAsync(yimg.p, 0xff, bo, s)); }
  pad2d_split(s, x1, (long long)H * W, Ci1, H, W, nullptr, 0, img.p, tp, g.margin);
  pad2d_split(s, x2, (long long)H * W, Ci2, H, W, nullptr, 0, img.p + b1, tp, g.margin);
  g.seg2_off = (long long)b1;
  ConvEpilogue e;
  if (yimg.p) { e.ys_out = yimg.p; e.ys_tp = tp; }
  { X3sForceScope force(ksplit, 0, 0); conv_x3s_run(L1, s, img.p, tp, (int)TP, yp.p, TP, e, &g); }
  unpad2d(s, yp.p, TP, Co, H, W, y, (long long)H * W);
  if (yimg.p) {
    split_image_to_f32(s, yimg.p + (size_t)(g.margin - kSplitMargin) * 16, tp, Co, (int)TP, yp.p, TP);
    unpad2d(s, yp.p, TP, Co, H, W, y_img_f32, (long long)H * W);
  }
  check_launch();
  RVC_HIP_CHECK(hipStreamSynchronize(s));
  RVC_CATCH
}
int rvc_op_gemm_split_swapped_res(void* stream, const float* x, const float* w, const float* res, float* y, int Ci, int Co, int T, int ld, int off) {
  RVC_TRY
  RVC_REQUIRE(x && w && res && y && Ci > 0 && Co > 0 && T > 0 && ld >= Co + off && off >= 0, "bad argument");
  hipStream_t s = (hipStream_t)stream;
  OwnedConvLayer L;
  { ConvBuildScope scope(2); conv1d_layer_init(L, w, nullptr, Co, Ci, 1, 1, 0, 1, 1); }
  DevBytes xs = image_from_f32(s, x, Ci, T, 0);
  conv_x3s_run_swapped(L, 0, Co, s, xs.p, split_image_tp(T), T, nullptr, 0, y + off, ld, res + off, ld);
  check_launch();
  RVC_HIP_CHECK(hipStreamSynchronize(s));
  RVC_CATCH
}
int rvc_op_attention_split(void* stream, const float* q, const float* k, const float* v, const float* bv, float* out, float* out_img_f32, int heads, int T) {
  RVC_TRY
  RVC_REQUIRE(q && k && v && (out || out_img_f32) && heads > 0 && T > 0, "bad argument");
  hipStream_t s = (hipStream_t)stream;
  const int C = heads * 64;
  DevBytes qk, vt, oi; DevBuf<float> vtf;
  const long long tp = split_image_tp(T);
  attention_operand_images(s, q, k, v, C, T, qk, vtf, vt);
  if (out_img_f32) oi.alloc(split_image_bytes(C, T));
  attention_split(s, qk.p, tp, 2 * C, 0, C / 16, vt.p, heads, 64, T, 1.f, bv, out, T, oi.p, tp);
  if (out_img_f32) split_image_to_f32(s, oi.p, tp, C, T, out_img_f32, T);
  check_launch();
  RVC_HIP_CHECK(hipStreamSynchronize(s));
  RVC_CATCH
}
int rvc_op_attention_split_rel(void* stream, const float* q, const float* k, const float* v, const float* bv, const float* ek_host, const float* ev_host,
                               float* out, float* out_img_f32, int heads, int T, int kz) {
  RVC_TRY
  RVC_REQUIRE(q && k && v && ek_host && ev_host && (out || out_img_f32) && heads > 0 && T > 0, "bad argument");
  hipStream_t s = (hipStream_t)stream;
  const int C = heads * 96;
  DevBytes qk, vt, oi, tab; DevBuf<float> vtf;
  std::vector<uint16_t> eki, evi;
  attention_rel_images(ek_host, ev_host, 96, 10, eki, evi);
  const size_t evt_off = eki.size() * 2;
  tab.alloc(evt_off + evi.size() * 2);
  RVC_HIP_CHECK(hipMemcpy(tab.p, eki.data(), evt_off, hipMemcpyHostToDevice));
  RVC_HIP_CHECK(hipMemcpy(tab.p + evt_off, evi.data(), evi.size() * 2, hipMemcpyHostToDevice));
  const long long tp = split_image_tp(T);
  attention_operand_images(s, q, k, v, C, T, qk, vtf, vt);
  if (out_img_f32) oi.alloc(split_image_bytes(C, T));
  { AttentionKzScope force(kz); attention_split(s, qk.p, tp, 2 * C, 0, C / 16, vt.p, heads, 96, T, 1.f, bv, out, T, oi.p, tp, 10, tab.p, tab.p + evt_off); }
  if (out_img_f32) split_image_to_f32(s, oi.p, tp, C, T, out_img_f32, T);
  check_launch();
  RVC_HIP_CHECK(hipStreamSynchronize(s));
  RVC_CATCH
}
int rvc_op_cbr2_small(void* stream, const float* x, const float* w1, const float* b1, const float* w2, const float* b2, float* y, int C, int H, int W) {
  RVC_TRY
  RVC_REQUIRE(x && w1 && b1 && w2 && b2 && y && (C == 16 || C == 32) && H > 0 && W > 0, "bad argument");
  hipStream_t s = (hipStream_t)stream;
// ... 305 lines not shown
  RVC_REQUIRE(in && out && R > 0 && C > 0 && batch > 0 && ldin >= C && ldout >= R, "bad argument");
  hipStream_t s = (hipStream_t)stream;
  transpose(s, in, out, R, C, ldin, ldout, batch, bin, bout);
  check_launch();
  RVC_HIP_CHECK(hipStreamSynchronize(s));
  RVC_CATCH
}
int rvc_op_frames(void* stream, const float* src, float* out, int L, int k, int stride, int pad, int Tout, int reflect) {
  RVC_TRY
  RVC_REQUIRE(src && out && L > 0 && k > 0 && stride > 0 && pad >= 0 && Tout > 0, "bad argument");
  RVC_REQUIRE(!reflect || (pad < L && (long long)(Tout - 1) * stride + k - 1 - pad <= 2LL * (L - 1)), "a reflected index must land inside the signal");
  hipStream_t s = (hipStream_t)stream;
  frames(s, src, out, L, k, stride, pad, Tout, reflect);
  check_launch();
  RVC_HIP_CHECK(hipStreamSynchronize(s));
  RVC_CATCH
}
int rvc_op_mel_to_unet(void* stream, const float* mel, float* x, int n, int Tr, float a, float b) {
  RVC_TRY
  RVC_REQUIRE(mel && x && n > 0 && Tr >= n && Tr <= 2 * n - 1, "bad argument (the right reflection must land inside the n frames)");
  hipStream_t s = (hipStream_t)stream;
  mel_to_unet(s, mel, x, n, Tr, a, b);
  check_launch();
  RVC_HIP_CHECK(hipStreamSynchronize(s));
  RVC_CATCH
}
int rvc_op_feats_prepare(void* stream, const float* f, const float* f0, const float* pitchf, float* out, int D, int Th, int T, float protect, int do_protect) {
  RVC_TRY
  RVC_REQUIRE(f && out && (pitchf || !do_protect) && D > 0 && Th > 0 && T > 0 && T <= 2 * Th, "bad argument");
  hipStream_t s = (hipStream_t)stream;
  feats_prepare(s, f, f0, pitchf, out, D, Th, T, protect, do_protect);
  check_launch();
  RVC_HIP_CHECK(hipStreamSynchronize(s));
  RVC_CATCH
}
int rvc_op_wn_gate(void* stream, const float* a, const float* g, float* out, float* out_img_f32, int H, int T) {
  RVC_TRY
  RVC_REQUIRE(a && g && (out || out_img_f32) && H > 0 && T > 0, "bad argument");
  hipStream_t s = (hipStream_t)stream;
  DevBytes img;
  if (out) wn_gate(s, a, g, out, H, T);
  if (out_img_f32) {
    const long long tp = split_image_tp(T);
    img.alloc(split_image_bytes(H, T));
    RVC_HIP_CHECK(hipMemsetAsync(img.p, 0xff, split_image_bytes(H, T), s));
    wn_gate_split(s, a, g, img.p, tp, kSplitMargin, H, T);
    split_image_to_f32(s, img.p, tp, H, T, out_img_f32, T);
  }
  check_launch();
  RVC_HIP_CHECK(hipStreamSynchronize(s));
  RVC_CATCH
}
int rvc_op_pool2_pad(void* stream, const float* x, int64_t ldx, int x_padded, int C, int H, int W, float* y, float* y_img_f32, int64_t ldy) {
  RVC_TRY
  RVC_REQUIRE(x && (y || y_img_f32) && C > 0 && H >= 2 && W >= 2, "bad argument");
  const int Ho = H / 2, Wo = W / 2; const long long P = (long long)Ho * (Wo + 2);
  RVC_REQUIRE(ldx >= (long long)H * (x_padded ? W + 2 : W) && ldy >= P, "bad pitch");
  hipStream_t s = (hipStream_t)stream;
  Image2d im;
  if (y_img_f32) im = image2d_alloc(s, C, Ho, Wo);
  pool2_pad_split(s, x, ldx, x_padded != 0, C, H, W, y, ldy, im.b.p, im.tp, im.margin);
  if (y_img_f32) image2d_to_f32(s, im, C, P, y_img_f32, ldy);
  check_launch();
  RVC_HIP_CHECK(hipStreamSynchronize(s));
  RVC_CATCH
}
int rvc_op_interleave2_pad(void* stream, const float* ph, int64_t ldp, int Co, int H, int W, float* y, int y_padded, float* y_img_f32, int64_t ldy) {
  RVC_TRY
  RVC_REQUIRE(ph && (y || y_img_f32) && Co > 0 && H > 0 && W > 0 && ldp >= (long long)H * (W + 2), "bad argument");
  const long long P = (long long)(2 * H) * (2 * W + 2);
  RVC_REQUIRE(ldy >= ((y_padded || y_img_f32) ? P : (long long)(2 * H) * (2 * W)), "bad pitch");
  hipStream_t s = (hipStream_t)stream;
  Image2d im;
  if (y_img_f32) im = image2d_alloc(s, Co, 2 * H, 2 * W);
  interleave2_pad_split(s, ph, ldp, Co, H, W, y, ldy, y_padded != 0, im.b.p, im.tp, im.margin);
  if (y_img_f32) image2d_to_f32(s, im, Co, P, y_img_f32, ldy);
  check_launch();
  RVC_HIP_CHECK(hipStreamSynchronize(s));
  RVC_CATCH
}
int rvc_op_pad2d(void* stream, const float* x, int64_t ldx, int C, int H, int W, float* y, float* y_img_f32, int64_t ldy) {
  RVC_TRY
  const long long P = (long long)H * (W + 2);
  RVC_REQUIRE(x && (y || y_img_f32) && C > 0 && H > 0 && W > 0 && ldx >= (long long)H * W && ldy >= P, "bad argument");
  hipStream_t s = (hipStream_t)stream;
  Image2d im;
  if (y_img_f32) im = image2d_alloc(s, C, H, W);
  pad2d_split(s, x, ldx, C, H, W, y, ldy, im.b.p, im.tp, im.margin);
  if (y_img_f32) image2d_to_f32(s, im, C, P, y_img_f32, ldy);
  check_launch();
  RVC_HIP_CHECK(hipStreamSynchronize(s));
  RVC_CATCH
}
int rvc_op_unpad2d(void* stream, const float* x, int64_t ldx, int C, int H, int W, float* y, int64_t ldy) {
  RVC_TRY
  RVC_REQUIRE(x && y && C > 0 && H > 0 && W > 0 && ldx >= (long long)H * (W + 2) && ldy >= (long long)H * W, "bad argument");
  hipStream_t s = (hipStream_t)stream;
  unpad2d(s, x, ldx, C, H, W, y, ldy);
  check_launch();
  RVC_HIP_CHECK(hipStreamSynchronize(s));
  RVC_CATCH
}
int rvc_op_gru_scan(void* stream, const float* gi, const float* b_ih, const float* w_hh, const float* b_hh, float* out, int T, int* err_out) {
  RVC_TRY
  RVC_REQUIRE(gi && b_ih && w_hh && b_hh && out && err_out && T > 0, "bad argument");
  hipStream_t s = (hipStream_t)stream;
  DevBuf<unsigned long long> xbuf; DevBuf<int> err;
  xbuf.alloc((size_t)2 * 2 * 256); err.alloc(2);
  gru_scan(s, gi, b_ih, w_hh, nullptr, b_hh, out, xbuf.p, err.p, T);
  check_launch();
  int e[2] = {0, 0};
  RVC_HIP_CHECK(hipMemcpyAsync(e, err.p, sizeof(e), hipMemcpyDeviceToHost, s));
  RVC_HIP_CHECK(hipStreamSynchronize(s));
  *err_out = e[0];
  RVC_CATCH
}

int rvc_prof_enable(int on) { RVC_TRY conv_prof_enable(on != 0); RVC_CATCH }
int rvc_set_conv_precision(int mode) {
  RVC_TRY
  RVC_REQUIRE(mode >= 0 && mode <= 2, "precision mode must be 0, 1 or 2");
  conv_set_precision(mode);
  RVC_CATCH
}
int rvc_set_pair_arithmetic(int mode) {
  RVC_TRY
  RVC_REQUIRE(mode == 0 || mode == 1, "pair arithmetic must be 0 (bf16x3) or 1 (fp16x2)");
  conv_set_pair_arithmetic(mode);
  RVC_CATCH
}
int rvc_get_pair_arithmetic(void) { return conv_set_pair_arithmetic(-1); }
int rvc_prof_collect(double* ms, double* flops, int64_t* launches) {
  RVC_TRY
  static_assert(RVC_PROF_CFGS == kProfCfgs, "profiling table size");
  long long l[RVC_PROF_CFGS];
  conv_prof_collect(ms, flops, l);
  for (int i = 0; i < RVC_PROF_CFGS; ++i) launches[i] = l[i];
  RVC_CATCH
}
int rvc_prof_collect_ex(double* out, double ridge_fp32, double ridge_x3) { RVC_TRY conv_prof_collect_ex(out, ridge_fp32, ridge_x3); RVC_CATCH }
const char* rvc_prof_cfg_name(int i) { return conv_prof_cfg_name(i); }
int rvc_prof_dump_csv(const char* path) { RVC_TRY RVC_REQUIRE(path && conv_prof_dump_csv(path) >= 0, "cannot write the launch table"); RVC_CATCH }
#ifdef RVC_EXPERIMENTS
int rvc_debug_read_scratch(void* stream, int slot, void* host_dst, size_t bytes) {
  RVC_TRY
  void* p = stream_scratch((hipStream_t)stream, slot, bytes);
  RVC_HIP_CHECK(hipStreamSynchronize((hipStream_t)stream));
  RVC_HIP_CHECK(hipMemcpy(host_dst, p, bytes, hipMemcpyDeviceToHost));
  RVC_CATCH
}
int rvc_debug_conv_timing(uint64_t* out8, int reset) { RVC_TRY conv_timing_read((unsigned long long*)out8, reset != 0); RVC_CATCH }
int rvc_debug_x3p_check(void) { return conv_x3p_check_read(); }
int rvc_debug_gemm_split_bench(void* stream, int Ci, int Co, int T, int ksplit, int am, int an, int split_out, int reps, float* us_out, int w2d, int nlayers) {
  RVC_TRY
  RVC_REQUIRE(us_out && reps > 0 && Ci > 0 && Co > 0 && T > 0 && nlayers >= 1 && nlayers <= 64, "bad argument");
  hipStream_t s = (hipStream_t)stream;
  const int kt = w2d > 0 ? 9 : 1;
  std::vector<float> w((size_t)Co * Ci * kt), b((size_t)Co, 0.01f);
  uint32_t st = 12345u;
  std::vector<OwnedConvLayer> Ls((size_t)nlayers);
  DevBuf<float> x, r, y; DevBytes xs, ys;
  struct Event { hipEvent_t e = nullptr; ~Event() { if (e) (void)hipEventDestroy(e); } } e0, e1;
  for (auto& L : Ls) {
    for (auto& v : w) { st = st * 1664525u + 1013904223u; v = ((float)(st >> 8) / 8388608.f - 1.f) * 0.05f; }
    ConvBuildScope scope(2);
    if (w2d > 0) conv2d3x3_layer_init(L, w.data(), b.data(), Co, Ci); else conv1d_layer_init(L, w.data(), b.data(), Co, Ci, 1, 1, 0, 1, 1);
  }
  SplitGeom g; if (w2d > 0) g = split_geom_2d(w2d);
  const long long tp = ((long long)g.margin + T + 704 + 63) & ~63LL;
  std::vector<float> hx((size_t)Ci * T);
  for (auto& v : hx) { st = st * 1664525u + 1013904223u; v = (float)(st >> 8) / 8388608.f - 1.f; }
  x.upload(hx);
  r.alloc((size_t)Co * T); RVC_HIP_CHECK(hipMemset(r.p, 0, (size_t)Co * T * 4));
  y.alloc((size_t)Co * T);
  const size_t ib = (size_t)(Ci / 16) * 4 * tp * 16, ob = (size_t)((Co + 15) / 16) * 4 * tp * 16;
  xs.alloc(ib); RVC_HIP_CHECK(hipMemset(xs.p, 0, ib)); ys.alloc(ob); RVC_HIP_CHECK(hipMemset(ys.p, 0, ob));
  split_image_from_f32(s, x.p, T, Ci, T, xs.p + (size_t)(g.margin - kSplitMargin) * 16, tp);
  ConvEpilogue e;
  if (split_out) { e.act = ACT_GELU; e.ys_out = ys.p; e.ys_tp = tp; } else { e.R = r.p; e.ldR = T; }
  X3sForceScope force(ksplit, am, an);
  for (auto& L : Ls) conv_x3s_run(L, s, xs.p, tp, T, split_out ? nullptr : y.p, T, e, w2d > 0 ? &g : nullptr);
  RVC_HIP_CHECK(hipEventCreate(&e0.e)); RVC_HIP_CHECK(hipEventCreate(&e1.e));
  RVC_HIP_CHECK(hipEventRecord(e0.e, s));
  for (int i = 0; i < reps; ++i) conv_x3s_run(Ls[(size_t)(i % nlayers)], s, xs.p, tp, T, split_out ? nullptr : y.p, T, e, w2d > 0 ? &g : nullptr);
  RVC_HIP_CHECK(hipEventRecord(e1.e, s));
  RVC_HIP_CHECK(hipEventSynchronize(e1.e));
  float ms = 0.f; RVC_HIP_CHECK(hipEventElapsedTime(&ms, e0.e, e1.e));
  *us_out = ms * 1e3f / (float)reps;
  RVC_CATCH
}

#endif

}
```

### comfy-rvc_amd/csrc/rvc_internal.h

```cpp
#pragma once
#include <atomic>
#include <hip/hip_runtime.h>
#include <cstdint>
#include <cstdio>
#include <cstdlib>
#include <cmath>
#include <cstring>
#include <map>
#include <mutex>
#include <string>
#include <vector>
#include <stdexcept>

namespace rvc {

void set_error(const std::string& msg);
struct Error : std::runtime_error { using std::runtime_error::runtime_error; };

#define RVC_HIP_CHECK(expr)                                                                       \
  do {                                                                                            \
    hipError_t _e = (expr);                                                                       \
    if (_e != hipSuccess)                                                                         \
      throw rvc::Error(std::string(#expr) + " failed: " + hipGetErrorString(_e) + " (" + __FILE__ + \
                       ":" + std::to_string(__LINE__) + ")");                                     \
  } while (0)

#define RVC_REQUIRE(cond, msg)                                                                    \
  do {                                                                                            \
    if (!(cond)) throw rvc::Error(std::string("requirement failed: ") + #cond + " : " + (msg));   \
  } while (0)

inline int knob_int(const char* name, int def) { const char* e = getenv(name); return e ? atoi(e) : def; }
#ifdef RVC_EXPERIMENTS
inline int exp_int(const char* name, int def) { return knob_int(name, def); }
#define RVC_EXP_STR(name) getenv(name)
#else
#define exp_int(name, def) (def)
#define RVC_EXP_STR(name) ((const char*)nullptr)
#endif

enum Act : int { ACT_NONE = 0, ACT_LRELU = 1, ACT_RELU = 2, ACT_GELU = 3, ACT_TANH = 4, ACT_SIGMOID = 5, ACT_LOGCLAMP = 6 };

struct ConvArgs {
  const float* X; const float* W; const float* bias; const float* R; float* Y;
  int Ci;
  int Co;
  int CoP;
  int Tin;
  int Tout;
  int Wd;
  int ktaps;
  int dil, stride, pad;
  int CK;
  int KT;
  int nchunk;
  int WROW;
  int PW, BWd, BH;
  long long xBatch, wBatch, yBatch, rBatch; int bBatch;
  long long ldX, ldY, ldR;
  int pre_act; float pre_slope;
  int act; float act_slope;
  int act_before_res;
  float out_scale; int accumulate;
  int ostride, orows;
  int up2;
  int KH, KW, PH, PWL;
};

struct ConvLayer {
  float* Wd_ = nullptr;
  float* bd_ = nullptr;
  float* bd4_ = nullptr;
  int mode = 1;
  int Ci = 0, Co = 0, CoP = 0, groups = 1;
  int k = 1, stride = 1, dil = 1, pad = 0;
  int ktaps = 1, CK = 8, KT = 1, nchunk = 1;
  int tconv_u = 0;
  int co_real = 0;
  int up2 = 0;
  int conv_pad = 0;
  long long wBatch = 0;
  int kh = 3, kw = 3, ph = 1, pwl = 1;
  uint16_t* Wx_ = nullptr;
  int CoPx = 0; long long wxBatch = 0;
  uint16_t* Wh_ = nullptr;
  int seg2_chunks = 0;
};

struct ConvEpilogue {
  const float* R = nullptr; long long ldR = 0;
  int pre_act = ACT_NONE; float pre_slope = 0.f;
  int act = ACT_NONE; float act_slope = 0.f;
  int act_before_res = 0;
  float out_scale = 1.f; int accumulate = 0;
  const float* bias_override = nullptr;
  int tout_limit = 0;
  int plan_tin = 0;
  const unsigned char* xs_in = nullptr; long long xs_tp = 0;
  unsigned char* ys_out = nullptr; long long ys_tp = 0; float ys_slope = 1.f;
  unsigned char* vt_out = nullptr; long long vt_tp = 0; int vt_row0 = 0;
  int gate_h = 0; const float* gate_g = nullptr;
  int ys_deint_h = 0;
  int h2 = 0;
};
constexpr int kSplitMargin = 64;
inline long long split_image_tp(long long T) { return (T + kSplitMargin + 704 + 63) & ~63LL; }
inline size_t split_image_bytes(int C, long long T) { return (size_t)(C / 16) * 2 * (size_t)split_image_tp(T) * 32; }
enum SplitRole : int { SPLIT_CONSUMER = 0, SPLIT_PRODUCER = 1 };
bool conv1d_split_eligible(const ConvLayer& L, int Tin, SplitRole role = SPLIT_CONSUMER, int h2 = 0);
bool conv1d_pair_h2_eligible(const ConvLayer& c1, const ConvLayer& c2, int Tin, int h2);
int conv1d_residual_period(const ConvLayer& L, int Tin, int h2);
int conv_set_pair_arithmetic(int mode);


void conv1d_layer_init(ConvLayer& L, const float* w , const float* bias, int Co, int Ci, int k,
                       int stride, int pad, int dil, int groups);
void tconv1d_layer_init(ConvLayer& L, const float* w , const float* bias, int Ci, int Co, int k, int u, int pad);
void conv2d3x3_layer_init(ConvLayer& L, const float* w , const float* bias, int Co, int Ci);
void conv2d1x1_layer_init(ConvLayer& L, const float* w , const float* bias, int Co, int Ci);
void tconv2d_layer_init(ConvLayer& L, const float* w , const float* bias, int Ci, int Co);
void conv2d_kx_layer_init(ConvLayer& L, const float* w , const float* bias, int Co, int Ci, int KH, int KW, int PH, int PWL);
bool conv_x3_set_default(bool on);
int conv_set_precision(int mode);
struct ConvBuildScope {
  int prev_mode; bool prev_default;
  explicit ConvBuildScope(int precision) : prev_mode(conv_set_precision(-1)), prev_default(conv_x3_set_default(true)) {
    if (precision >= 0) conv_set_precision(precision);
  }
  ~ConvBuildScope() { conv_x3_set_default(prev_default); conv_set_precision(prev_mode); }
  ConvBuildScope(const ConvBuildScope&) = delete; ConvBuildScope& operator=(const ConvBuildScope&) = delete;
};

int conv1d_out_len(const ConvLayer& L, int Tin);
void conv1d_run(const ConvLayer& L, hipStream_t s, const float* X, long long ldX, int Tin, float* Y, long long ldY,
                const ConvEpilogue& e);
void gemm_tn_run(hipStream_t s, const float* A, long long ldA, long long aBatch, const float* B, long long ldB, long long bBatch,
                 float* Y, long long ldY, long long yBatch, int M, int N, int K, int batch, const float* bias, int biasBatch,
                 const ConvEpilogue& e);
void conv2d_run(const ConvLayer& L, hipStream_t s, const float* X, long long ldX, int H, int Wd, float* Y, long long ldY,
                const ConvEpilogue& e);

struct SplitGeom { int ktaps = 1; int toff[16] = {0}; int padw = 0; int margin = kSplitMargin;
                   long long seg2_off = 0;
                   int s2_h = 0; };
void conv_layer_append_x3(ConvLayer& dst, const ConvLayer& extra);
SplitGeom split_geom_2d(int Wd, int KH = 3, int KW = 3, int PH = 1, int PWL = 1);
inline int split_s2_h(long long Tin) { return (int)(((Tin + 1) / 2 + 64 + 63) & ~63LL); }
inline long long split_s2_tp(long long Tin) { return (kSplitMargin + 2LL * split_s2_h(Tin) + 704 + 63) & ~63LL; }
inline size_t split_s2_bytes(int C, long long Tin) { return (size_t)(C / 16) * 2 * (size_t)split_s2_tp(Tin) * 32; }
SplitGeom split_geom_s2(int k, long long Tin);
bool conv_x3s_s2_eligible(const ConvLayer& L);
inline int wn_gate_row_order(int p, int H) { const int b = p >> 5, q = p & 31; return q < 16 ? 16 * b + q : H + 16 * b + (q - 16); }
void split_image_deint_from_f32(hipStream_t s, const float* X, long long ldX, int C, int T, unsigned char* img, long long tp, int H);
void split_image_deint_to_f32(hipStream_t s, const unsigned char* img, long long tp, int H, int C, int T, float* Y, long long ldY);
bool conv_x3s_eligible(const ConvLayer& L);
void conv_x3s_run(const ConvLayer& L, hipStream_t s, const unsigned char* Xs, long long xsTp, int T, float* Y, long long ldY, const ConvEpilogue& e,
                  const SplitGeom* geom = nullptr);
void conv_x3s_run_swapped(const ConvLayer& L, int row0, int rows, hipStream_t s, const unsigned char* Xs, long long xsTp, int T, unsigned char* Ys, long long ysTp,
                          float* Yrm = nullptr, long long ldYrm = 0,
                          const float* Rrm = nullptr, long long ldRrm = 0);
void split_image_from_tm(hipStream_t s, const float* x, int C, int T, int M, unsigned char* img, long long tp);
void conv_x3s_force(int ksplit, int am, int an);
void x3_weight_image(const float* w, int Co, int Ci, int k, int CoPx, std::vector<uint16_t>& P);
struct ConvX3dArgs {
  const float* X; const unsigned char* Wx; const float* bias; float* Y;
  int Ci, Co, CoPx, H, Hout, p, k, stride, pad, S; float slope;
};
struct ConvX3dPlan { ConvX3dArgs a; dim3 grid; int units = 1; size_t lds = 0; double flops = 0.0; };
bool conv_x3d_plan(const ConvX3dArgs& a, ConvX3dPlan& p);
void conv_x3d_launch(const ConvX3dPlan& p, hipStream_t s);
struct ConvX3dBwdArgs {
  const float* D; const unsigned char* Wx[3]; const float* Cot; const float* A; float* Y;
  int R, RPx, Ck, Hd, H, p, ostride, off0, nph, S; int nt[3]; int Hj[3]; int tile0[4]; float slope;
};
struct ConvX3dBwdPlan { ConvX3dBwdArgs a; dim3 grid; int units = 1; size_t lds = 0; double flops = 0.0; };
bool conv_x3d_bwd_plan(const ConvX3dBwdArgs& a, ConvX3dBwdPlan& p);
void conv_x3d_bwd_launch(const ConvX3dBwdPlan& p, hipStream_t s);
struct ConvGenBwdArgs {
  const float* D; long long ldD; int Td; const unsigned char* Wx; const float* A; const float* Res; float* Y; long long ldY;
  int R, RPx, Ck, N, nt, cstride, tstep, off0; float slope, scale; int accumulate;
};
struct ConvGenBwdPlan { ConvGenBwdArgs a; dim3 grid; int bm = 128, units = 1; size_t lds = 0; double flops = 0.0; };
bool conv_gen_bwd_plan(const ConvGenBwdArgs& a, ConvGenBwdPlan& p);
void conv_gen_bwd_launch(const ConvGenBwdPlan& p, hipStream_t s);
void gen_tanh_bwd(hipStream_t s, const float* dy, const float* y, float* d, long long n);
void gen_post_bwd(hipStream_t s, const float* d, const float* w, const float* x, float* dx, int C, int k, int pad, long long T, float slope, float scale);
void gen_noise_bwd(hipStream_t s, const float* D, const float* w, float* dhar, float* out2, int C, int k, int stride, int pad, long long T, long long N, int accumulate);
void gen_row_sums(hipStream_t s, const float* D, int C, long long T, float* out, float* out2);
void gen_cond_bwd(hipStream_t s, const float* W, const float* dcond, int C, int G, float* out, float* out2);
struct ConvX3dWgradArgs {
  const float* D; const float* X; float* part;
  int Ci, Co, H, Hout, p, k, stride, pad, S; int cps, per, total;
};
struct ConvX3dWgradPlan { ConvX3dWgradArgs a; dim3 grid; int splits = 1; size_t lds = 0, part_floats = 0; double flops = 0.0; };
bool conv_x3d_wgrad_plan(const ConvX3dWgradArgs& a, ConvX3dWgradPlan& p);
void conv_x3d_wgrad_launch(const ConvX3dWgradPlan& p, hipStream_t s);
constexpr int kGenWgradMaxItems = 16;
constexpr size_t kGenWgradPartFloats = (size_t)16 << 20;
struct GenItems { const float* p[kGenWgradMaxItems]; };
struct ConvGenWgradArgs {
  const float* P[kGenWgradMaxItems]; const float* G[kGenWgradMaxItems]; float* part;
  int B, R, C, k, N; long long ldP, ldG; int Tg, cstride, tstep, off0; float slopeP, slopeG; int cps, per, total;
};
struct ConvGenWgradPlan { ConvGenWgradArgs a; dim3 grid; int bm = 128, splits = 1; size_t lds = 0, part_floats = 0; double flops = 0.0; };
bool conv_gen_wgrad_plan(const ConvGenWgradArgs& a, ConvGenWgradPlan& p);
void conv_gen_wgrad_launch(const ConvGenWgradPlan& p, hipStream_t s);
struct GenWgradFinishArgs { const float* part; long long pstride; int splits, R, L; const float* v; const float* g; float* gw; float* gg; float* gb; GenItems D; int B, brows; long long N; };
void gen_wgrad_finish(hipStream_t s, const GenWgradFinishArgs& a);
void gen_wgrad_noise(hipStream_t s, const GenItems& D, const GenItems& H, int B, int C, long long T, long long Nh, int k, int stride, int pad, float* gw, float* gb);
void gen_wgrad_post(hipStream_t s, const GenItems& D, const GenItems& X, int B, int C, long long T, int k, int pad, float slope, float* gw);
void gen_wgrad_cond(hipStream_t s, const GenItems& DC, const GenItems& Gv, int B, int C, int G, float* gw, float* gb, float* gb2);
void gen_wgrad_msource(hipStream_t s, const GenItems& DH, const GenItems& H, const GenItems& Sn, int B, long long N, float* gw, float* gb);
bool cbr2_small_eligible(const ConvLayer& c1, const ConvLayer& c2);
void cbr2_small_run(const ConvLayer& c1, const ConvLayer& c2, hipStream_t s, const float* x, int H, int W, float* out);
bool conv3_small_eligible(const ConvLayer& L);
void conv3_small_run(const ConvLayer& L, hipStream_t s, const float* x, int H, int W, float* Y, float* Y2, int split_row, int relu_rows, const float* R);
void split_image_from_f32(hipStream_t s, const float* X, long long ldX, int C, int T, unsigned char* img, long long tp);
void split_image_to_f32(hipStream_t s, const unsigned char* img, long long tp, int C, int T, float* Y, long long ldY);

void attention_fused(hipStream_t s, const float* Q, const float* K, long long ldqk, const float* V, long long ldv, const float* bv,
                     float* out, long long ldo, int heads, int dhead, int T, unsigned char* out_img = nullptr, long long img_tp = 0);

long long attention_vt_tp(int channels);
size_t attention_vt_bytes(int channels, int T);
void attention_vt_clear_tail(hipStream_t s, unsigned char* vt_img, int channels, int T);
void attention_split(hipStream_t s, const unsigned char* qk_img, long long qk_tp, int qk_channels, int q_chunk0, int k_chunk0, const unsigned char* vt_img,
                     int heads, int dhead, int T, float scale, const float* bv, float* out, long long ldo, unsigned char* out_img, long long img_tp,
                     int win = 0, const unsigned char* ek_img = nullptr, const unsigned char* evt_img = nullptr);
void attention_split_force_kz(int kz);
void attention_rel_images(const float* ek, const float* ev, int D, int win, std::vector<uint16_t>& ek_img, std::vector<uint16_t>& evt_img);
void attention_rel_fused(hipStream_t s, const float* Q, const float* K, long long ldqk, const float* V, long long ldv, const float* bv,
                         const float* rel, float* pb, int win, float* out, long long ldo, int heads, int dhead, int T, const float* ek = nullptr,
                         const float* ev = nullptr);

void conv_prof_enable(bool on);
int conv_prof_collect(double* ms, double* flops, long long* launches);
const char* conv_prof_cfg_name(int i);
void conv_timing_read(unsigned long long* out8, bool reset);

void* dev_alloc(size_t bytes);
void* dev_upload(const void* host, size_t bytes);
template <typename T> T* dev_upload(const T* host, size_t n) { return static_cast<T*>(dev_upload(static_cast<const void*>(host), n * sizeof(T))); }
void dev_free(void* p);
void* stream_scratch(hipStream_t s, int slot, size_t bytes);
void* stream_scratch_zeroed(hipStream_t s, int slot, size_t bytes, bool* fresh = nullptr);
void stream_scratch_release(int device);

template <typename T> struct DevBuf {
  T* p = nullptr; size_t n = 0;
  DevBuf() = default;
  ~DevBuf() { dev_free(p); }
  DevBuf(DevBuf&& o) noexcept : p(o.p), n(o.n) { o.p = nullptr; o.n = 0; }
  DevBuf& operator=(DevBuf&& o) noexcept { if (this != &o) { dev_free(p); p = o.p; n = o.n; o.p = nullptr; o.n = 0; } return *this; }
  DevBuf(const DevBuf&) = delete; DevBuf& operator=(const DevBuf&) = delete;
  T* get() const { return p; }
  void reset() { dev_free(p); p = nullptr; n = 0; }
  void alloc(size_t cnt) { reset(); p = static_cast<T*>(dev_alloc(cnt * sizeof(T))); n = cnt; }
  void upload(const T* h, size_t cnt) { reset(); p = dev_upload(h, cnt); n = cnt; }
  void upload(const std::vector<T>& h) { upload(h.data(), h.size()); }
};

struct OwnedConvLayer : ConvLayer {
  OwnedConvLayer() = default;
  ~OwnedConvLayer() { free_weights(); }
  OwnedConvLayer(OwnedConvLayer&& o) noexcept : ConvLayer(o) { o.disown(); }
  OwnedConvLayer& operator=(OwnedConvLayer&& o) noexcept { if (this != &o) { free_weights(); ConvLayer::operator=(o); o.disown(); } return *this; }
  OwnedConvLayer(const OwnedConvLayer&) = delete; OwnedConvLayer& operator=(const OwnedConvLayer&) = delete;
  OwnedConvLayer(const ConvLayer&) = delete; OwnedConvLayer& operator=(const ConvLayer&) = delete;
 private:
  void disown() { Wd_ = bd_ = bd4_ = nullptr; Wx_ = Wh_ = nullptr; }
  void free_weights() { dev_free(Wd_); dev_free(bd_); dev_free(bd4_); dev_free(Wx_); dev_free(Wh_); }
};

#define RVC_ALLOW_BIG_LDS(kern)                                                                                                              \
  do {                                                                                                                                       \
    static std::atomic<unsigned long long> rvc_lds_mask_[4];                                                                                 \
    int rvc_dev_ = 0; (void)hipGetDevice(&rvc_dev_);                                                                                         \
    const unsigned long long rvc_bit_ = 1ull << (rvc_dev_ & 63);                                                                             \
    std::atomic<unsigned long long>& rvc_m_ = rvc_lds_mask_[(rvc_dev_ >> 6) & 3];                                                            \
    if (!(rvc_m_.load(std::memory_order_acquire) & rvc_bit_)) {                                                                              \
      RVC_HIP_CHECK(hipFuncSetAttribute(reinterpret_cast<const void*>(kern), hipFuncAttributeMaxDynamicSharedMemorySize, 160 * 1024));      \
      rvc_m_.fetch_or(rvc_bit_, std::memory_order_release);                                                                                  \
    }                                                                                                                                        \
  } while (0)

struct Arena {
  char* base = nullptr; size_t cap = 0, off = 0, peak = 0; bool dry = false;
  unsigned gen = 0;
  void reset() { off = 0; }
  template <typename T> T* alloc(size_t n) {
    size_t bytes = (n * sizeof(T) + 255) & ~size_t(255);
    size_t o = off; off += bytes; if (off > peak) peak = off;
    if (dry) return reinterpret_cast<T*>(uintptr_t(0x1000) + o);
    RVC_REQUIRE(off <= cap, "arena overflow");
    return reinterpret_cast<T*>(base + o);
  }
  void ensure(size_t bytes);
  void release();
  Arena() = default;
  ~Arena() { release(); }
  Arena(const Arena&) = delete; Arena& operator=(const Arena&) = delete;
};

template <typename F> void arena_passes(Arena& A, F&& graph) {
  struct Restore { Arena& a; ~Restore() { a.dry = false; } } restore{A};
  A.dry = true; A.reset(); A.peak = 0;
  graph();
  A.ensure(A.peak);
  A.dry = false; A.reset();
  graph();
}

struct ZeroedBlock {
  const void* base = nullptr; unsigned gen = 0; size_t bytes = 0; int key0 = -1, key1 = -1;
  bool stale(const void* b, unsigned g, size_t n, int k0, int k1) const { return base != b || gen != g || bytes != n || key0 != k0 || key1 != k1; }
// ... 11 lines not shown
```

### include/rvc_hip.h

```cpp
#ifndef RVC_HIP_H
#define RVC_HIP_H
#include <stdint.h>

#ifdef __cplusplus
extern "C" {
#endif

typedef struct rvc_ctx rvc_ctx;
typedef struct rvc_hubert rvc_hubert;
typedef struct rvc_rmvpe rvc_rmvpe;
typedef struct rvc_synth rvc_synth;

const char* rvc_last_error(void);
const char* rvc_version(void);

int rvc_ctx_create(int device_id, rvc_ctx** out);
int rvc_ctx_destroy(rvc_ctx* ctx);
int64_t rvc_ctx_workspace_bytes(rvc_ctx* ctx);
int rvc_ctx_set_conv_precision(rvc_ctx* ctx, int mode);

typedef struct rvc_hubert_taps {
  float* conv_stack;
  float* pos_conv;
  float* hidden_0;
// ... 96 lines not shown

int rvc_synth_has_posterior(rvc_synth* s);
typedef struct rvc_synth_forward_taps {
  float* z; float* z_p; float* m_p; float* logs_p; float* m_q; float* logs_q;
} rvc_synth_forward_taps;
int rvc_synth_forward(rvc_synth* s, void* stream, const float* phone_dev, int phone_channel_major, const int64_t* pitch_dev, const float* pitchf_dev,
                      const float* spec_dev, int sid, const float* noise_q_dev, const float* noise_src_dev, int64_t T, int64_t ids, float* out_dev,
                      const rvc_synth_forward_taps* taps);
typedef struct rvc_gen_tape rvc_gen_tape;
int rvc_gen_tape_create(rvc_synth* s, rvc_gen_tape** out);
int rvc_gen_tape_release(rvc_gen_tape* t);
int64_t rvc_gen_tape_bytes(rvc_gen_tape* t);
int rvc_gen_tape_tensor(rvc_gen_tape* t, const char* name, float** ptr_dev, int* rows, int64_t* cols);
int rvc_gen_tape_timing(rvc_gen_tape* t, int on);
int rvc_gen_tape_times(rvc_gen_tape* t, float* ms_host, int cap);
int rvc_synth_forward_tape(rvc_synth* s, void* stream, const float* phone_dev, int phone_channel_major, const int64_t* pitch_dev, const float* pitchf_dev,
                           const float* spec_dev, int sid, const float* noise_q_dev, const float* noise_src_dev, int64_t T, int64_t ids, float* out_dev,
                           const rvc_synth_forward_taps* taps, rvc_gen_tape* tape);
int rvc_synth_dec_input_grad(rvc_synth* s, void* stream, rvc_gen_tape* tape, const float* dy_hat_dev, float* dz_dev, float* dcond_dev, float* dg_dev,
                             float* dhar_dev);
int rvc_synth_dec_input_grad_launch_count(rvc_synth* s);
int rvc_synth_keep_parameters(rvc_synth* s, int on);
int rvc_synth_dec_param_count(rvc_synth* s);
int rvc_synth_dec_param_info(rvc_synth* s, int k, char* name, int name_cap, int64_t* shape, int* ndim);
int64_t rvc_synth_dec_param_total(rvc_synth* s);
int rvc_synth_dec_weight_grad(rvc_synth* s, void* stream, rvc_gen_tape* const* tapes, int B, float* const* grads_dev);
int rvc_synth_dec_weight_grad_launch_count(rvc_synth* s);
int rvc_gen_tape_wgrad_times(rvc_gen_tape* t, float* ms_host, int cap);
int rvc_conv1d_weight_grad(void* stream, const float* const* p_dev, const float* const* g_dev, int B, int R, int C, int k, int64_t N, int64_t Tg, int cstride,
                           int tstep, int off0, float slope_p, float slope_g, float* out_dev);
int rvc_conv1d_weight_grad_splits(int B, int R, int C, int k, int64_t N, int64_t Tg, int cstride, int tstep, int off0);
int rvc_kl_loss(void* stream, const float* z_p_dev, const float* logs_q_dev, const float* m_p_dev, const float* logs_p_dev, int C, int64_t T_pitch,
                int64_t len, double* sum_dev);
int rvc_kl_loss_grad(void* stream, const float* z_p_dev, const float* m_p_dev, const float* logs_p_dev, int C, int64_t T_pitch, int64_t len, float scale,
                     float* dz_p_dev, float* dlogs_q_dev, float* dm_p_dev, float* dlogs_p_dev);
int rvc_l1_sum(void* stream, const float* a_dev, const float* b_dev, int64_t n, double* sum_dev);

typedef struct rvc_disc rvc_disc;
int rvc_disc_create(rvc_ctx* ctx, int version, rvc_disc** out);
int rvc_disc_set_tensor(rvc_disc* d, const char* name, const float* host_data, const int64_t* shape, int ndim);
int rvc_disc_finalize(rvc_disc* d);
int rvc_disc_release(rvc_disc* d);
int rvc_disc_count(rvc_disc* d);
int rvc_disc_num_taps(rvc_disc* d, int i);
int rvc_disc_tap_shape(rvc_disc* d, int i, int tap, int64_t T, int* C, int* H, int* p);
int rvc_disc_forward(rvc_disc* d, void* stream, const float* signals_dev, int S, int64_t T, float* const* scores_dev, float* const* fmaps_dev);
int rvc_disc_launch_count(rvc_disc* d, int S, int64_t T);
int rvc_sqerr_sums(void* stream, const float* const* x_dev, const int64_t* n, const float* c, int K, double* sums_dev);
int rvc_l1_sums(void* stream, const float* const* a_dev, const float* const* b_dev, const int64_t* n, int K, double* sums_dev);
int rvc_disc_input_grad(rvc_disc* d, void* stream, int S, int64_t T, const float* const* fmaps_dev, const float* const* dtaps_dev, float* const* work_dev,
                        float* dsignals_dev);
int rvc_disc_input_grad_launch_count(rvc_disc* d, int S, int64_t T);
int rvc_disc_keep_parameters(rvc_disc* d, int on);
int rvc_disc_param_count(rvc_disc* d);
int rvc_disc_param_info(rvc_disc* d, int k, char* name, int name_cap, int64_t* shape, int* ndim);
int rvc_disc_weight_grad(rvc_disc* d, void* stream, const float* signals_dev, int S, int64_t T, const float* const* fmaps_dev,
                         const float* const* deltas_dev, float* const* grads_dev);
int rvc_disc_weight_grad_launch_count(rvc_disc* d, int S, int64_t T);
typedef struct rvc_adamw_hyper {
  double lr, beta1, beta2, eps, weight_decay;
  int64_t step;
  int has_clip;
  double clip_value;
} rvc_adamw_hyper;
int rvc_adamw_step(void* stream, float* const* p_dev, const float* const* g_dev, float* const* m_dev, float* const* v_dev, const int64_t* n, int K,
                   const rvc_adamw_hyper* hyper);
int rvc_disc_adamw_step(rvc_disc* d, void* stream, const float* grads_flat_dev, float* exp_avg_flat_dev, float* exp_avg_sq_flat_dev, const rvc_adamw_hyper* hyper);
int rvc_disc_adamw_step_launch_count(rvc_disc* d);
int64_t rvc_disc_param_total(rvc_disc* d);
int rvc_disc_get_parameters(rvc_disc* d, void* stream, float* flat_dev);
int rvc_disc_set_parameters(rvc_disc* d, void* stream, const float* flat_dev);
int rvc_loss_cotangents(void* stream, int kind, const float* const* a_dev, const float* const* b_dev, const int64_t* n, const float* scale, int K,
                        float* const* out_dev);
int rvc_interpolate(void* stream, const float* alpha_dev, const float* y_dev, const float* y_hat_dev, int B, int64_t T, float* out_dev);

int rvc_vc_segment(rvc_hubert* h, rvc_synth* s, void* stream, const float* audio_dev, int64_t L, int version,
                   const int64_t* pitch_dev, const float* pitchf_dev, int sid, float protect, int do_protect,
                   const float* noise_z_dev, const float* noise_src_dev, float* out_dev);

int rvc_vc_segment_feats(rvc_synth* s, void* stream, const float* feats_cm_dev, const float* feats0_cm_dev, int64_t T_h, int feat_dim,
                         const int64_t* pitch_dev, const float* pitchf_dev, int sid, float protect, int do_protect,
                         const float* noise_z_dev, const float* noise_src_dev, float* out_dev);
int rvc_vc_segment_window(rvc_hubert* h, rvc_synth* s, void* stream, const float* audio_dev, int64_t L, int version,
                          const int64_t* pitch_dev, const float* pitchf_dev, int sid, float protect, int do_protect,
                          const float* noise_z_dev, const float* noise_src_dev, float* out_dev, int64_t keep0, int64_t keep1);
int rvc_vc_segment_feats_window(rvc_synth* s, void* stream, const float* feats_cm_dev, const float* feats0_cm_dev, int64_t T_h, int feat_dim,
                                const int64_t* pitch_dev, const float* pitchf_dev, int sid, float protect, int do_protect,
                                const float* noise_z_dev, const float* noise_src_dev, float* out_dev, int64_t keep0, int64_t keep1);

typedef struct rvc_index rvc_index;
int rvc_index_create(rvc_ctx* ctx, const float* big_npy_host, int64_t N, int D, rvc_index** out);
int rvc_index_create_ivf(rvc_ctx* ctx, const float* big_npy_host, int64_t N, int D, const float* centroids_host , int nlist,
                         const int32_t* list_of_host , int nprobe, rvc_index** out);
int rvc_index_nprobe(const rvc_index* h);
int rvc_index_destroy(rvc_index* h);
int64_t rvc_index_ntotal(const rvc_index* h);
int rvc_index_search(rvc_index* h, void* stream, const float* feats_cm_dev, int64_t T, int64_t* idx_dev, float* score_dev );
int rvc_index_blend(rvc_index* h, void* stream, const float* feats_cm_dev, const int64_t* idx_dev, int64_t T, float index_rate, float* out_cm_dev);
int rvc_kmeans_assign(rvc_ctx* ctx, void* stream, const float* rows_dev, int64_t N, int D, const float* cent_dev , int K, int32_t* label_dev,
                      float* dist_dev );
int rvc_kmeans_update(void* stream, const float* rows_dev, const int32_t* label_dev, int64_t N, int D, int K, float* cent_dev ,
                      int32_t* count_dev);
int rvc_index_train(rvc_ctx* ctx, void* stream, const float* rows_dev, int64_t N, int D, const int64_t* init_rows_host , int K, int niter,
                    float* cent_dev , int32_t* label_dev, double* inertia_host );
int rvc_preprocess(void* stream, const void* audio_dev, int is_f64, int64_t n, const double* b6_host, const double* a6_host,
                   const double* zi5_host, int t_pad, double* filt_dev, float* padded_dev, double* rms1_dev, int n1,
                   const double* sos18_host, const double* sos_zi6_host);
int rvc_postprocess(void* stream, float* wav_dev, int64_t N, const double* rms1_dev, int n1, int sr2, float rms_mix_rate, int16_t* out_i16_dev);

int rvc_lfilter_hp(void* stream, const void* x_dev, int is_f64, int64_t n, const double* sos18_host, double* y_dev);
int rvc_frame_rms(void* stream, const double* x_dev, int64_t n, int win, int hop, double* rms_dev, int64_t n_frames);
int rvc_slice_tags(const double* rms_host, int64_t n_frames, int64_t n_samples, double threshold, int64_t min_length, int64_t min_interval,
                   int64_t max_sil_kept, int64_t* tags_host, int64_t cap, int64_t* n_tags);
int rvc_cut_windows(void* stream, const double* filt_dev, int64_t n, const int64_t* windows_dev, int n_windows, int sr, int target_sr,
                    const double* taps_dev, int half, int up, int down, float max_volume, float* gt_dev, int64_t total_gt, float* y16_dev,
                    int64_t total_16);

int rvc_gate_levels(void* stream, const float* x_dev, int64_t n, int win, double* ss_dev, int64_t n_windows);
int rvc_gate_ranges(const double* level_db_host, int64_t n_windows, int64_t n, int64_t win, int64_t min_size, int64_t fade, double threshold_db,
                    int64_t* ranges_host, int64_t cap, int64_t* n_ranges);
int rvc_gate_apply(void* stream, const float* x_dev, float* y_dev, int64_t n, const int64_t* ranges_dev, int n_ranges, int64_t fade);
int rvc_declick(void* stream, const float* x_dev, int64_t n, int size, float multiplier, int method, int kernel_size, int detect, float* y_dev,
                uint8_t* mask_dev);
int rvc_peak_normalize(void* stream, const float* x_dev, int64_t n, float gain, float* y_dev);
int rvc_peak_limit(void* stream, float* x_dev, int64_t n, float max_volume);
int rvc_merge_tracks(void* stream, const float* const* tracks_host, const int64_t* lens_host, int k, int mode, float* out_dev, int64_t n_out);
int rvc_segment_energy(void* stream, const int16_t* x_dev, int64_t n, int k, int64_t* out_dev);

int rvc_spectrogram_batch(rvc_ctx* ctx, void* stream, const float* audio_dev, int64_t n_audio, const int64_t* clips_host, int n_clips, int n_fft, int hop,
                          float eps, int clamp, float* out_dev, int64_t pitch);
int rvc_mel_filterbank_set(rvc_ctx* ctx, int n_fft, int n_mels, const int32_t* first_host, const int32_t* count_host, const float* weights_host);
int rvc_spec_to_mel_batch(rvc_ctx* ctx, void* stream, const float* spec_dev, int64_t spec_pitch, const int64_t* clips_host, int n_clips, int n_fft,
                          int n_mels, float* mel_dev, int64_t mel_pitch);
int rvc_spectrogram_batch_ms(rvc_ctx* ctx, void* stream, const float* audio_dev, int64_t n_audio, const int64_t* clips_host, int n_clips, int n_fft, int hop,
                             float eps, int clamp, float* out_dev, int64_t pitch);
int rvc_mel_spectrogram_vjp(rvc_ctx* ctx, void* stream, const float* audio_dev, int64_t n_audio, const int64_t* clips_host, int n_clips, int n_fft, int hop,
                            float eps, int clamp, int n_mels, const float* cot_mel_dev, int64_t pitch, float* d_audio_dev);
int rvc_mel_spectrogram_vjp_launch_count(void);
int rvc_mel_loss_cotangents(void* stream, int K, const float* const* a_dev, const float* const* b_dev, const int64_t* n, int loss, float log_weight,
                            float mag_weight, const float* scale, float* const* out_dev);
int rvc_multiscale_mel_loss(rvc_ctx* ctx, void* stream, int K, const float* const* spec_dev, const int64_t* pitch, const int64_t* row_stride, int B, int64_t nf,
                            const int32_t* n_fft, const int32_t* n_mels, int loss, int want_mag, double* out_dev);

int rvc_hpss(void* stream, const float* x_dev, int B, int F, int T, float* h_dev, float* p_dev, int medians);
int rvc_hpss_l1(void* stream, const float* org_dev, const float* gen_dev, int B, int F, int T, float eps, double* sums_dev);
int rvc_tsi_terms(void* stream, const float* org_dev, const float* gen_dev, int B, int F, int T, float eps, double* out_dev);

int rvc_op_conv1d(void* stream, const float* x_dev, const float* w_host, const float* bias_host, const float* res_dev, float* y_dev,
                  int Ci, int Co, int Tin, int k, int stride, int pad, int dil, int groups, int pre_act, float pre_slope, int act,
                  float act_slope, int act_before_res, float out_scale, int accumulate);
int rvc_op_gemm_split(void* stream, const float* x_dev, const float* w_host, const float* bias_host, const float* res_dev, float* y_dev,
                      float* ysplit_f32_dev, int Ci, int Co, int T, int act, float act_slope, int act_before_res, float out_scale, int ksplit,
                      int am, int an, int k, int dil);
int rvc_op_conv1d_split(void* stream, const float* x_dev, const float* w_host, const float* bias_host, const float* res_dev, float* y_dev,
                        int Ci, int Co, int T, int k, int pad, int dil, int groups, int act, int act_before_res);
int rvc_op_conv1d_s2_split(void* stream, const float* x_dev, const float* w_host, const float* bias_host, float* y_dev, float* y_img_f32_dev, int Ci, int Co, int T, int k,
                           int act);
int rvc_op_conv2d_split(void* stream, const float* x_dev, const float* w_host, const float* bias_host, const float* res_dev, float* y_dev,
                        float* ysplit_f32_dev, int Ci, int Co, int H, int W, int act, int act_before_res, int ksplit, int am, int an);
int rvc_op_conv_transpose1d(void* stream, const float* x_dev, const float* w_host, const float* bias_host, float* y_dev, int Ci, int Co,
                            int Tin, int k, int u, int pad, int pre_act, float pre_slope, int accumulate);
int rvc_op_conv2d3x3(void* stream, const float* x_dev, const float* w_host, const float* bias_host, const float* res_dev, float* y_dev,
                     int Ci, int Co, int H, int W, int relu);
int rvc_op_conv_transpose2d(void* stream, const float* x_dev, const float* w_host, const float* bias_host, float* y_dev, int Ci, int Co,
                            int H, int W, int relu);
int rvc_op_gemm_tn(void* stream, const float* a_dev, const float* b_dev, float* y_dev, int M, int N, int K, int batch);
typedef struct rvc_conv1d_plan rvc_conv1d_plan;
int rvc_conv1d_plan_create(const float* w_host, const float* bias_host, int Ci, int Co, int k, int stride, int pad, int dil, int groups,
                           rvc_conv1d_plan** out);
int rvc_conv1d_plan_run(rvc_conv1d_plan* p, void* stream, const float* x_dev, int Tin, const float* res_dev, float* y_dev, int pre_act,
                        float pre_slope, int act, float act_slope);
int rvc_conv1d_plan_pair_split_run(rvc_conv1d_plan* c1, rvc_conv1d_plan* c2, void* stream, const float* x_dev, int T, float* y_dev,
                                   float out_scale, int accumulate);
int rvc_conv1d_plan_pair_run(rvc_conv1d_plan* c1, rvc_conv1d_plan* c2, void* stream, const float* x_dev, int T, float* y_dev, float out_scale,
                             int accumulate);
int rvc_conv1d_plan_resblock_run(rvc_conv1d_plan* const* plans6, void* stream, const float* x_dev, int T, float* y_dev, float out_scale, int accumulate,
                                 int* ran_out, const float* noise_src_dev, const float* noise_w_dev, const float* noise_b_dev);
int rvc_conv1d_plan_pair_arithmetic(rvc_conv1d_plan* c1, rvc_conv1d_plan* c2, int T);
int rvc_conv1d_plan_destroy(rvc_conv1d_plan* p);
int rvc_op_attention(void* stream, const float* q_dev, const float* k_dev, const float* v_rm_dev, const float* bv_dev, float* out_dev,
                     int heads, int T);
int rvc_op_attention_split(void* stream, const float* q_dev, const float* k_dev, const float* v_dev, const float* bv_dev, float* out_dev,
                           float* out_img_f32_dev, int heads, int T);
int rvc_op_attention_split_rel(void* stream, const float* q_dev, const float* k_dev, const float* v_dev, const float* bv_dev, const float* ek_host,
                               const float* ev_host, float* out_dev, float* out_img_f32_dev, int heads, int T, int kz);
int rvc_op_cbr2_small(void* stream, const float* x_dev, const float* w1_host, const float* b1_host, const float* w2_host, const float* b2_host,
                      float* y_dev, int C, int H, int W);
int rvc_op_layernorm_c_split(void* stream, const float* x_dev, const float* gamma_dev, const float* beta_dev, float* y_dev, float* y_img_f32_dev, int C, int T);
int rvc_op_conv3_small(void* stream, const float* x_dev, const float* w_host, const float* b_host, const float* res_dev, float* y_dev, float* y2_dev, int Ci, int Co,
                       int H, int W, int split_row, int relu_rows);
int rvc_op_wn_in_gate_split(void* stream, const float* x_dev, const float* w_host, const float* bias_host, const float* g_dev, float* y_dev, int Ci, int H, int T, int k);
int rvc_op_gemm_split_qkv(void* stream, const float* x_dev, const float* w_host, const float* bias_host, float* y_img_f32_dev, float* yt_dev, int Ci, int Co, int T,
                          int vt_row0);
int rvc_op_gemm_split_swapped(void* stream, const float* x_dev, const float* w_host, float* yt_dev, int Ci, int Co, int T, int row0, int rows);
int rvc_op_conv2d3x3_plus_1x1(void* stream, const float* x1_dev, const float* w1_host, const float* x2_dev, const float* w2_host, float* y_dev, float* y_img_f32_dev,
                              int Ci1, int Ci2, int Co, int H, int W, int ksplit);
int rvc_op_gemm_split_swapped_res(void* stream, const float* x_dev, const float* w_host, const float* res_dev, float* y_dev, int Ci, int Co, int T, int ld, int off);
int rvc_op_attention_rel(void* stream, const float* q_dev, const float* k_dev, const float* v_rm_dev, const float* bv_dev, const float* rel_dev,
                         float* pb_dev, float* out_dev, int heads, int T, const float* ek_dev, const float* ev_dev);
int rvc_op_layernorm_c(void* stream, const float* x_dev, const float* res_dev, const float* gamma_dev, const float* beta_dev, float* y_dev,
                       int C, int T);
int rvc_op_sine_source(void* stream, const float* f0_dev, const float* noise_dev, float* har_dev, float* sine_dev, int T, int upp, float sr,
                       float lin_w, float lin_b, float* rad_dev, float* tmp_dev, float* phase_dev);

int rvc_op_hubert_conv0(void* stream, const float* audio_dev, int64_t L, const float* w_dev, const float* gamma_dev, const float* beta_dev, int C, int T1,
                        float* out_dev, float* out_img_f32_dev, int64_t ld);
int rvc_op_conv_to1(void* stream, const float* x_dev, int64_t ldx, const float* w_dev, int Ci, int K, int pad, int T, float pre_slope, int act_tanh, float* y_dev,
                    int* kernel_out);
int rvc_op_noise_add(void* stream, float* x_dev, int64_t ld, int C, int T, const float* src_dev, int64_t L, int k, int stride, int pad, const float* w_dev,
                     const float* b_dev, int* ran_out);
int rvc_op_transpose(void* stream, const float* in_dev, float* out_dev, int R, int C, int64_t ldin, int64_t ldout, int batch, int64_t bin, int64_t bout);
int rvc_op_frames(void* stream, const float* src_dev, float* out_dev, int L, int k, int stride, int pad, int Tout, int reflect);
int rvc_op_mel_to_unet(void* stream, const float* mel_dev, float* x_dev, int n, int Tr, float a, float b);
int rvc_op_feats_prepare(void* stream, const float* f_dev, const float* f0_dev, const float* pitchf_dev, float* out_dev, int D, int Th, int T, float protect,
                         int do_protect);
int rvc_op_wn_gate(void* stream, const float* a_dev, const float* g_dev, float* out_dev, float* out_img_f32_dev, int H, int T);
int rvc_op_pool2_pad(void* stream, const float* x_dev, int64_t ldx, int x_padded, int C, int H, int W, float* y_dev, float* y_img_f32_dev, int64_t ldy);
int rvc_op_interleave2_pad(void* stream, const float* ph_dev, int64_t ldp, int Co, int H, int W, float* y_dev, int y_padded, float* y_img_f32_dev, int64_t ldy);
int rvc_op_pad2d(void* stream, const float* x_dev, int64_t ldx, int C, int H, int W, float* y_dev, float* y_img_f32_dev, int64_t ldy);
int rvc_op_unpad2d(void* stream, const float* x_dev, int64_t ldx, int C, int H, int W, float* y_dev, int64_t ldy);
int rvc_op_gru_scan(void* stream, const float* gi_dev, const float* b_ih_dev, const float* w_hh_dev, const float* b_hh_dev, float* out_dev, int T, int* err_out);

int rvc_resample(void* stream, const float* x_dev, int64_t n_in, const double* taps_dev, int half, int up, int down, float* y_dev, int64_t n_out);

int rvc_set_conv_precision(int mode);
int rvc_set_pair_arithmetic(int mode);
int rvc_get_pair_arithmetic(void);

#define RVC_PROF_CFGS 24
int rvc_prof_enable(int on);
int rvc_prof_collect(double* ms, double* flops, int64_t* launches);
int rvc_prof_collect_ex(double* out, double ridge_fp32, double ridge_bf16x3);
const char* rvc_prof_cfg_name(int i);
int rvc_prof_dump_csv(const char* path);
#ifdef RVC_EXPERIMENTS
int rvc_debug_conv_timing(uint64_t* out8, int reset);
int rvc_debug_x3p_check(void);
int rvc_debug_gemm_split_bench(void* stream, int Ci, int Co, int T, int ksplit, int am, int an, int split_out, int reps, float* us_out, int w2d,
                               int nlayers);

#endif

#ifdef __cplusplus
}
#endif
#endif
```

Baseline: 2395 audio-sec/wall-sec.

## Add two-team intra-workgroup K-split to x3s conv GEMM kernel

Adds a TEAMS=2 variant of the split-bf16 conv GEMM kernel. Two 4-wave teams in one 512-thread workgroup each process half of the K units in their own LDS ring, and team 1's accumulators are merged into team 0's through LDS. The planner enables it by default for 64-wide tiles with few units per slice, halving the global K-split where possible. This replaces cross-workgroup slab reductions with an in-LDS merge. In exchange it doubles LDS per block and lowers occupancy.

```diff
diff --git a/comfy-rvc_amd/_lib.py b/comfy-rvc_amd/_lib.py
--- a/comfy-rvc_amd/_lib.py
+++ b/comfy-rvc_amd/_lib.py
@@ -214,6 +214,7 @@
     "rvc_hpss_l1": (c_int, [c_void_p, c_void_p, c_void_p, c_int, c_int, c_int, c_float, c_void_p]),
     "rvc_tsi_terms": (c_int, [c_void_p, c_void_p, c_void_p, c_int, c_int, c_int, c_float, c_void_p]),
     "rvc_op_gemm_split": (c_int, [c_void_p] * 7 + [c_int] * 4 + [c_float, c_int, c_float] + [c_int] * 5),
+    "rvc_op_gemm_split_teams": (c_int, [c_void_p] * 7 + [c_int] * 4 + [c_float, c_int, c_float] + [c_int] * 6),
     "rvc_op_conv2d_split": (c_int, [c_void_p] * 7 + [c_int] * 9),
     "rvc_op_wn_in_gate_split": (c_int, [c_void_p] * 6 + [c_int] * 4),
     "rvc_op_gemm_split_qkv": (c_int, [c_void_p] * 6 + [c_int] * 4),
@@ -272,6 +273,7 @@
     "rvc_debug_conv_timing": (c_int, [P(C.c_uint64), c_int]),
     "rvc_debug_x3p_check": (c_int, []),
     "rvc_debug_gemm_split_bench": (c_int, [c_void_p] + [c_int] * 8 + [P(c_float), c_int, c_int]),
+    "rvc_debug_gemm_split_bench_teams": (c_int, [c_void_p] + [c_int] * 8 + [P(c_float), c_int, c_int, c_int]),
 }
 
 for _name, (_res, _args) in SIGNATURES.items():
diff --git a/comfy-rvc_amd/csrc/conv_x3s.hip b/comfy-rvc_amd/csrc/conv_x3s.hip
--- a/comfy-rvc_amd/csrc/conv_x3s.hip
+++ b/comfy-rvc_amd/csrc/conv_x3s.hip
@@ -33,20 +33,25 @@
 
 RVC_PHASE_TABLE_REGISTER;
 
-constexpr int x3s_wgs(int AM, int AN, int RS) { return (AM * AN >= 4 && RS != 3) ? 2 : 3; }
-template <int AM, int AN, int RS>
-__global__ __launch_bounds__(256, x3s_wgs(AM, AN, RS)) void conv_x3s_kernel(const GemmSArgs p) {
+constexpr int x3s_wgs(int AM, int AN, int RS, int TEAMS = 1) { return TEAMS == 2 ? 2 : (AM * AN >= 4 && RS != 3) ? 2 : 3; }
+template <int AM, int AN, int RS, int TEAMS = 1>
+__global__ __launch_bounds__(256 * TEAMS, x3s_wgs(AM, AN, RS, TEAMS)) void conv_x3s_kernel(const GemmSArgs p) {
   constexpr int WN = 2, NW = 4;
+  static_assert(TEAMS == 1 || TEAMS == 2, "one or two wave teams");
   constexpr int BM = 64 * AM, BN = 64 * AN;
   constexpr int NPA = BM / 16, NPB = BN / 16, NPW = (NPA + NPB) / NW;
   static_assert((NPA % NW) == 0 && (NPB % NW) == 0, "every wave's i-th piece is of one kind");
   constexpr int aslot = BM * 64, bslot = BN * 64, uslot = aslot + bslot;
   static_assert(RS >= 3 && (RS - 2) * NPW <= 63, "ring");
+  constexpr int ring_bytes = RS * uslot;
+  static_assert(TEAMS == 1 || (AM * AN * 16384 <= ring_bytes && ring_bytes >= 1024 + NW * 4096), "merge buffer inside team 1's ring, clear of the flag word and the V^T scratch");
   extern __shared__ __attribute__((aligned(1024))) unsigned char smem3s[];
 
   const int tid0 = threadIdx.x;
   int lane = tid0 & 63;
-  const int wave = __builtin_amdgcn_readfirstlane(tid0 >> 6);
+  const int wave8 = __builtin_amdgcn_readfirstlane(tid0 >> 6);
+  const int team = TEAMS == 2 ? wave8 >> 2 : 0, wave = TEAMS == 2 ? wave8 & 3 : wave8;
+  unsigned char* const ring = smem3s + team * ring_bytes;
   const int wm = wave / WN, wn = wave % WN;
   const int li = lane & 31, lh = lane >> 5;
   const unsigned total = gridDim.x;
@@ -57,13 +62,14 @@
   const int grp = tile_y / p.rows_pg;
   const int co0 = (tile_y - grp * p.rows_pg) * BM, n0 = tile_x * BN;
   const int row0 = grp * p.co_g, CoG = p.co_g;
-  const int U1 = p.nunits / S, u0 = ks * U1;
+  const int kse = ks * TEAMS + team;
+  const int U1 = p.nunits / (S * TEAMS), u0 = kse * U1;
   PhaseTimer<PhaseClock::cycle> tm;
   tm.add(0, 1);
 
   const bool r_pre = p.R != nullptr && !(p.act_before_res && p.act != ACT_NONE);
   f32x16 acc[AM][AN];
-  if (ks == 0 && (p.bias != nullptr || r_pre)) {
+  if (kse == 0 && (p.bias != nullptr || r_pre)) {
     const __amdgpu_buffer_rsrc_t rrs = make_rsrc(r_pre ? p.R : (const float*)p.Wx, r_pre ? (unsigned)(p.groups * p.co_g) * (unsigned)p.ldR * 4u : 0u);
 #pragma unroll
     for (int am = 0; am < AM; ++am)
@@ -114,7 +120,7 @@
   const int seg2_at = p.seg2_u - u0;
   int slw = 0, uw = 0;
   auto issue = [&]() {
-    unsigned char* base = smem3s + slw * uslot;
+    unsigned char* base = ring + slw * uslot;
 #pragma unroll
     for (int i = 0; i < NPW; ++i) {
       if (i * NW < NPA) buf_dma(ars, base + dsto[i], voff[i], soff_a);
@@ -150,8 +156,8 @@
   struct Ops { u32x4 ah[AM], al[AM], bh[AN], bl[AN]; };
   Ops o0, o1;
   auto read_ops = [&](Ops& o, int slot_i) {
-    const unsigned char* wa = smem3s + slot_i * uslot + aoff;
-    const unsigned char* xa = smem3s + slot_i * uslot + boff;
+    const unsigned char* wa = ring + slot_i * uslot + aoff;
+    const unsigned char* xa = ring + slot_i * uslot + boff;
 #pragma unroll
     for (int am = 0; am < AM; ++am) { o.ah[am] = *reinterpret_cast<const u32x4*>(wa + am * 512); o.al[am] = *reinterpret_cast<const u32x4*>(wa + BM * 32 + am * 512); }
 #pragma unroll
@@ -196,6 +202,38 @@
   tm.lap(2);
   asm volatile("s_waitcnt vmcnt(0)" ::: "memory");
   tm.mark();
+  const bool vt_tile = co0 >= p.vt_row0;
+  if (TEAMS == 2 || vt_tile) lds_barrier();
+  if constexpr (TEAMS == 2) {
+    constexpr int QM = AM * AN * 4;
+    unsigned char* mrg = smem3s + ring_bytes + ((wave * QM * 64) + lane) * 16;
+    if (team == 1) {
+#pragma unroll
+      for (int am = 0; am < AM; ++am)
+#pragma unroll
+        for (int an = 0; an < AN; ++an)
+#pragma unroll
+          for (int q = 0; q < 4; ++q)
+            *reinterpret_cast<u32x4*>(mrg + ((am * AN + an) * 4 + q) * 1024) = u32x4{__float_as_uint(acc[am][an][4 * q]), __float_as_uint(acc[am][an][4 * q + 1]),
+                                                                                      __float_as_uint(acc[am][an][4 * q + 2]), __float_as_uint(acc[am][an][4 * q + 3])};
+    }
+    lds_barrier();
+    if (team == 0) {
+#pragma unroll
+      for (int am = 0; am < AM; ++am)
+#pragma unroll
+        for (int an = 0; an < AN; ++an)
+#pragma unroll
+          for (int q = 0; q < 4; ++q) {
+            const u32x4 v = *reinterpret_cast<const u32x4*>(mrg + ((am * AN + an) * 4 + q) * 1024);
+#pragma unroll
+            for (int j = 0; j < 4; ++j) acc[am][an][4 * q + j] = acc[am][an][4 * q + j] + __uint_as_float(v[j]);
+          }
+    } else if (S == 1) {
+      tm.lap(5); tm.flush();
+      return;
+    }
+  }
 
   if (S > 1) {
     typedef float f32x4_t __attribute__((ext_vector_type(4)));
@@ -203,7 +241,7 @@
     const unsigned slab_bytes = 256u * QN * 16u;
     const __amdgpu_buffer_rsrc_t srs = make_rsrc(p.slabs, (unsigned)(total) * slab_bytes);
     const unsigned lane_off = ((unsigned)wave * QN * 64u + (unsigned)lane) * 16u;
-    {
+    if (team == 0) {
       const unsigned mine = ((unsigned)tile * (unsigned)S + (unsigned)ks) * slab_bytes + lane_off;
 #pragma unroll
       for (int am = 0; am < AM; ++am)
@@ -226,7 +264,7 @@
     }
     __syncthreads();
     tm.lap(5); tm.flush();
-    if (*flag != (unsigned)S - 1u) return;
+    if (*flag != (unsigned)S - 1u || team != 0) return;
 #pragma unroll
     for (int am = 0; am < AM; ++am)
 #pragma unroll
@@ -304,7 +342,6 @@
       }
     }
   }
-  const bool vt_tile = co0 >= p.vt_row0;
   if (vt_tile) {
     typedef float f32x4v __attribute__((ext_vector_type(4)));
     unsigned char* tl = smem3s + 1024 + wave * 4096;
@@ -546,14 +583,19 @@
   hipLaunchKernelGGL(unsplit_image_kernel, dim3((T + 255) / 256, (C + 15) / 16 * 2), dim3(256), 0, s, img, tp, C, T, Y, ldY);
 }
 
-template <int AM, int AN, int RS>
+template <int AM, int AN, int RS, int TEAMS = 1>
 static void launch_x3s(const GemmSArgs& a, unsigned blocks, hipStream_t s) {
-  auto kern = conv_x3s_kernel<AM, AN, RS>;
-  constexpr size_t lds = (size_t)RS * (64 * AM + 64 * AN) * 64;
+  auto kern = conv_x3s_kernel<AM, AN, RS, TEAMS>;
+  constexpr size_t lds = (size_t)TEAMS * RS * (64 * AM + 64 * AN) * 64;
   RVC_ALLOW_BIG_LDS(kern);
-  conv_launch(kern, dim3(blocks), dim3(256), lds, s, a);
-}
-static void x3s_dispatch(const GemmSArgs& a, int AM, int AN, unsigned blocks, hipStream_t s) {
+  conv_launch(kern, dim3(blocks), dim3(256 * TEAMS), lds, s, a);
+}
+static void x3s_dispatch(const GemmSArgs& a, int AM, int AN, int TEAMS, unsigned blocks, hipStream_t s) {
+  if (TEAMS == 2) {
+    RVC_REQUIRE(AN == 1 && a.nunits % (2 * a.ksplit) == 0, "conv_x3s: two teams want a 64 x 64 or 128 x 64 tile and an even unit count per slice");
+    if (AM == 2) launch_x3s<2, 1, 3, 2>(a, blocks, s); else launch_x3s<1, 1, 4, 2>(a, blocks, s);
+    return;
+  }
   const bool rs3 = AM == 2 && AN == 2 && blocks >= 768u && a.nunits / a.ksplit >= 64;
   if (AM == 2 && AN == 2) { if (rs3) launch_x3s<2, 2, 3>(a, blocks, s); else launch_x3s<2, 2, 4>(a, blocks, s); }
   else if (AM == 2 && AN == 1) launch_x3s<2, 1, 4>(a, blocks, s);
@@ -561,9 +603,9 @@
   else launch_x3s<1, 1, 4>(a, blocks, s);
 }
 
-static thread_local int t_force_s = 0, t_force_am = 0, t_force_an = 0;
-void conv_x3s_force(int ksplit, int am, int an) { t_force_s = ksplit; t_force_am = am; t_force_an = an; }
-static void x3s_plan(int M, long long Nplan, int units, int& AM, int& AN, int& S, int groups = 1) {
+static thread_local int t_force_s = 0, t_force_am = 0, t_force_an = 0, t_force_teams = 0;
+void conv_x3s_force(int ksplit, int am, int an, int teams) { t_force_s = ksplit; t_force_am = am; t_force_an = an; t_force_teams = teams; }
+static void x3s_plan(int M, long long Nplan, int units, int& AM, int& AN, int& S, int& TEAMS, int groups = 1) {
   static const int target = exp_int("RVC_X3S_BLK", 440);
   auto tiles = [&](int am, int an) { return (long long)groups * ((M + 64 * am - 1) / (64 * am)) * ((Nplan + 64 * an - 1) / (64 * an)); };
   AM = 2; AN = 2;
@@ -581,6 +623,18 @@
     if (units % c == 0 && units / c >= min_units) S = c;
   }
   if (t_force_s > 0) S = (units % t_force_s == 0 && units / t_force_s >= 4) ? t_force_s : 1;
+  TEAMS = 1;
+  static const int teams_on = exp_int("RVC_X3S_TEAMS", 1), team_units = exp_int("RVC_X3S_TEAMUNITS", 6), team_max = exp_int("RVC_X3S_TEAMMAX", 64);
+  constexpr long long kTeamSlots = 2 * 256;
+  const bool team_tile = AN == 1 && (AM == 1 || t_force_teams == 2);
+  auto teams_fit = [&](int s, int lo, int hi) { return team_tile && units % (2 * s) == 0 && units / (2 * s) >= lo && units / (2 * s) <= hi; };
+  if (t_force_teams == 2) {
+    if (teams_fit(S, 4, units)) TEAMS = 2;
+  } else if (t_force_teams == 0 && teams_on) {
+    auto lo = [&](long long wgs) { return wgs <= 256 ? team_units : std::max(team_units, 8); };
+    if (t_force_s == 0 && (S & 1) == 0 && teams_fit(S / 2, lo(nt * (S / 2)), team_max) && nt * (S / 2) <= kTeamSlots) { S /= 2; TEAMS = 2; }
+    else if (teams_fit(S, lo(nt * S), team_max) && nt * S <= kTeamSlots) TEAMS = 2;
+  }
 }
 
 bool conv_x3s_eligible(const ConvLayer& L) {
@@ -670,8 +724,8 @@
   a.groups = G; a.co_g = L.Co; a.cig_chunks = L.Ci / 16; a.wg_bytes = (unsigned)((double)(L.Ci / 16) * geom->ktaps * 4.0 * (double)L.CoPx * 16.0);
   a.bias = e.bias_override ? e.bias_override : L.bd_; a.R = e.R; a.ldR = e.ldR; a.Y = Y; a.ldY = ldY; a.Ys = e.ys_out; a.ysTp = e.ys_tp;
   a.act = e.act; a.act_slope = e.act_slope; a.act_before_res = e.act_before_res; a.out_scale = e.out_scale;
-  int AM, AN, S;
-  x3s_plan(L.Co, e.plan_tin > 0 ? e.plan_tin : T, a.nunits, AM, AN, S, G);
+  int AM, AN, S, TEAMS;
+  x3s_plan(L.Co, e.plan_tin > 0 ? e.plan_tin : T, a.nunits, AM, AN, S, TEAMS, G);
   const int BM = 64 * AM, BN = 64 * AN;
   RVC_REQUIRE(L.CoPx % BM == 0, "weight image rows are padded to the tile");
   a.rows_pg = (L.Co + BM - 1) / BM;
@@ -688,7 +742,7 @@
     a.slabs = (float*)stream_scratch(s, 6, slab_bytes);
   }
   ProfTicket tk = conv_prof_begin(s);
-  x3s_dispatch(a, AM, AN, blocks, s);
+  x3s_dispatch(a, AM, AN, TEAMS, blocks, s);
   if (tk.on) {
     ConvArgsX pa{};
     pa.Ci = L.Ci; pa.Co = L.Co; pa.ktaps = geom->ktaps; pa.kreal = geom->ktaps; pa.dil = L.mode == 1 ? L.dil : 1; pa.stride = s2 ? 2 : 1; pa.Tin = T; pa.Tout = T;
@@ -717,8 +771,8 @@
   a.Ys = Ys; a.ysTp = ysTp; a.act = ACT_NONE; a.out_scale = 1.f;
   a.Y = Yrm; a.ldY = ldYrm;
   a.R = Rrm; a.ldR = ldRrm;
-  int AM, AN, S;
-  x3s_plan(T, rows, a.nunits, AM, AN, S);
+  int AM, AN, S, TEAMS;
+  x3s_plan(T, rows, a.nunits, AM, AN, S, TEAMS);
   S = 1;
   const int BM = 64 * AM, BN = 64 * AN;
   RVC_REQUIRE((long long)((T + BM - 1) / BM) * BM <= xsTp - kSplitMargin && (long long)row0 + (long long)((rows + BN - 1) / BN) * BN <= L.CoPx, "conv_x3s_run_swapped: a tile would read past an operand image");
@@ -726,7 +780,7 @@
   a.xcd_remap = x3_xcd_remap();
   const unsigned blocks = (unsigned)((long long)a.gx * a.gy);
   ProfTicket tk = conv_prof_begin(s);
-  x3s_dispatch(a, AM, AN, blocks, s);
+  x3s_dispatch(a, AM, AN, TEAMS, blocks, s);
   if (tk.on) {
     ConvArgsX pa{};
     pa.Ci = L.Ci; pa.Co = rows; pa.ktaps = 1; pa.kreal = 1; pa.dil = 1; pa.stride = 1; pa.Tin = T; pa.Tout = T; pa.ksplit = 1;
diff --git a/comfy-rvc_amd/csrc/rvc_api.hip b/comfy-rvc_amd/csrc/rvc_api.hip
--- a/comfy-rvc_amd/csrc/rvc_api.hip
+++ b/comfy-rvc_amd/csrc/rvc_api.hip
@@ -24,8 +24,8 @@
   catch (...) { rvc::set_error("unknown error"); return 2; }
 
 struct X3sForceScope {
-  X3sForceScope(int ksplit, int am, int an) { conv_x3s_force(ksplit, am, an); }
-  ~X3sForceScope() { conv_x3s_force(0, 0, 0); }
+  X3sForceScope(int ksplit, int am, int an, int teams = 0) { conv_x3s_force(ksplit, am, an, teams); }
+  ~X3sForceScope() { conv_x3s_force(0, 0, 0, 0); }
   X3sForceScope(const X3sForceScope&) = delete; X3sForceScope& operator=(const X3sForceScope&) = delete;
 };
 struct AttentionKzScope {
@@ -924,8 +924,12 @@
 }
 int rvc_op_gemm_split(void* stream, const float* x, const float* w, const float* bias, const float* res, float* y, float* ysplit_f32, int Ci, int Co,
                       int T, int act, float act_slope, int act_before_res, float out_scale, int ksplit, int am, int an, int k, int dil) {
-  RVC_TRY
-  RVC_REQUIRE(x && w && (y || ysplit_f32) && Ci > 0 && Co > 0 && T > 0 && k >= 1 && (k & 1) == 1 && dil >= 1, "bad argument");
+  return rvc_op_gemm_split_teams(stream, x, w, bias, res, y, ysplit_f32, Ci, Co, T, act, act_slope, act_before_res, out_scale, ksplit, am, an, k, dil, 0);
+}
+int rvc_op_gemm_split_teams(void* stream, const float* x, const float* w, const float* bias, const float* res, float* y, float* ysplit_f32, int Ci, int Co,
+                            int T, int act, float act_slope, int act_before_res, float out_scale, int ksplit, int am, int an, int k, int dil, int teams) {
+  RVC_TRY
+  RVC_REQUIRE(x && w && (y || ysplit_f32) && Ci > 0 && Co > 0 && T > 0 && k >= 1 && (k & 1) == 1 && dil >= 1 && teams >= 0 && teams <= 2, "bad argument");
   hipStream_t s = (hipStream_t)stream;
   OwnedConvLayer L;
   { ConvBuildScope scope(2); conv1d_layer_init(L, w, bias, Co, Ci, k, 1, (k - 1) / 2 * dil, dil, 1); }
@@ -934,7 +938,7 @@
   DevBytes xs = image_from_f32(s, x, Ci, T, 0), ys;
   ConvEpilogue e; e.act = act; e.act_slope = act_slope; e.act_before_res = act_before_res; e.out_scale = out_scale; e.R = res; e.ldR = T;
   if (ysplit_f32) { ys.alloc(split_image_bytes(Co, T)); e.ys_out = ys.p; e.ys_tp = tp; }
-  { X3sForceScope force(ksplit, am, an); conv_x3s_run(L, s, xs.p, tp, T, y, T, e); }
+  { X3sForceScope force(ksplit, am, an, teams); conv_x3s_run(L, s, xs.p, tp, T, y, T, e); }
   if (ysplit_f32) split_image_to_f32(s, ys.p, tp, Co, T, ysplit_f32, T);
   check_launch();
   RVC_HIP_CHECK(hipStreamSynchronize(s));
@@ -1546,6 +1550,9 @@
 int rvc_debug_conv_timing(uint64_t* out8, int reset) { RVC_TRY conv_timing_read((unsigned long long*)out8, reset != 0); RVC_CATCH }
 int rvc_debug_x3p_check(void) { return conv_x3p_check_read(); }
 int rvc_debug_gemm_split_bench(void* stream, int Ci, int Co, int T, int ksplit, int am, int an, int split_out, int reps, float* us_out, int w2d, int nlayers) {
+  return rvc_debug_gemm_split_bench_teams(stream, Ci, Co, T, ksplit, am, an, split_out, reps, us_out, w2d, nlayers, 0);
+}
+int rvc_debug_gemm_split_bench_teams(void* stream, int Ci, int Co, int T, int ksplit, int am, int an, int split_out, int reps, float* us_out, int w2d, int nlayers, int teams) {
   RVC_TRY
   RVC_REQUIRE(us_out && reps > 0 && Ci > 0 && Co > 0 && T > 0 && nlayers >= 1 && nlayers <= 64, "bad argument");
   hipStream_t s = (hipStream_t)stream;
@@ -1572,7 +1579,7 @@
   split_image_from_f32(s, x.p, T, Ci, T, xs.p + (size_t)(g.margin - kSplitMargin) * 16, tp);
   ConvEpilogue e;
   if (split_out) { e.act = ACT_GELU; e.ys_out = ys.p; e.ys_tp = tp; } else { e.R = r.p; e.ldR = T; }
-  X3sForceScope force(ksplit, am, an);
+  X3sForceScope force(ksplit, am, an, teams);
   for (auto& L : Ls) conv_x3s_run(L, s, xs.p, tp, T, split_out ? nullptr : y.p, T, e, w2d > 0 ? &g : nullptr);
   RVC_HIP_CHECK(hipEventCreate(&e0.e)); RVC_HIP_CHECK(hipEventCreate(&e1.e));
   RVC_HIP_CHECK(hipEventRecord(e0.e, s));
diff --git a/comfy-rvc_amd/csrc/rvc_internal.h b/comfy-rvc_amd/csrc/rvc_internal.h
--- a/comfy-rvc_amd/csrc/rvc_internal.h
+++ b/comfy-rvc_amd/csrc/rvc_internal.h
@@ -160,7 +160,7 @@
                           float* Yrm = nullptr, long long ldYrm = 0,
                           const float* Rrm = nullptr, long long ldRrm = 0);
 void split_image_from_tm(hipStream_t s, const float* x, int C, int T, int M, unsigned char* img, long long tp);
-void conv_x3s_force(int ksplit, int am, int an);
+void conv_x3s_force(int ksplit, int am, int an, int teams = 0);
 void x3_weight_image(const float* w, int Co, int Ci, int k, int CoPx, std::vector<uint16_t>& P);
 struct ConvX3dArgs {
   const float* X; const unsigned char* Wx; const float* bias; float* Y;
diff --git a/include/rvc_hip.h b/include/rvc_hip.h
--- a/include/rvc_hip.h
+++ b/include/rvc_hip.h
@@ -272,6 +272,9 @@
 int rvc_op_gemm_split(void* stream, const float* x_dev, const float* w_host, const float* bias_host, const float* res_dev, float* y_dev,
                       float* ysplit_f32_dev, int Ci, int Co, int T, int act, float act_slope, int act_before_res, float out_scale, int ksplit,
                       int am, int an, int k, int dil);
+int rvc_op_gemm_split_teams(void* stream, const float* x_dev, const float* w_host, const float* bias_host, const float* res_dev, float* y_dev,
+                            float* ysplit_f32_dev, int Ci, int Co, int T, int act, float act_slope, int act_before_res, float out_scale, int ksplit,
+                            int am, int an, int k, int dil, int teams);
 int rvc_op_conv1d_split(void* stream, const float* x_dev, const float* w_host, const float* bias_host, const float* res_dev, float* y_dev,
                         int Ci, int Co, int T, int k, int pad, int dil, int groups, int act, int act_before_res);
 int rvc_op_conv1d_s2_split(void* stream, const float* x_dev, const float* w_host, const float* bias_host, float* y_dev, float* y_img_f32_dev, int Ci, int Co, int T, int k,
@@ -358,6 +361,8 @@
 int rvc_debug_x3p_check(void);
 int rvc_debug_gemm_split_bench(void* stream, int Ci, int Co, int T, int ksplit, int am, int an, int split_out, int reps, float* us_out, int w2d,
                                int nlayers);
+int rvc_debug_gemm_split_bench_teams(void* stream, int Ci, int Co, int T, int ksplit, int am, int an, int split_out, int reps, float* us_out, int w2d,
+                                     int nlayers, int teams);
 
 #endif
 
```

Result: no change. 2405 audio-sec/wall-sec, median of 4 (+0.4%).
